# VinAIResearch/GaPro

Hardware: AMD Instinct MI355X
Metric: scenes/sec pseudo-label gen (ScanNetV2-train-shaped synthetic scenes) (higher is better)
Workload: dtype f64

## Files before the change

### gapro_amd/_lib.py

```python
from __future__ import annotations

import ctypes as C
import os
import sys
from typing import Optional

_HERE = os.path.dirname(os.path.abspath(__file__))
LIB_PATH = os.path.join(_HERE, "libgapro_hip.so")

GAPRO_OK = 0
GAPRO_ERR_BAD_ARG = -1
GAPRO_ERR_NOT_FINITE = -4
GAPRO_ERR_CHOLESKY = -5
STATUS_NAMES = {0: "OK", -1: "BAD_ARG", -2: "OOM", -3: "HIP", -4: "NOT_FINITE", -5: "CHOLESKY", -6: "SPP_RANGE",
                -7: "WORKSPACE", -8: "TIMEOUT", -9: "IO", -10: "UNSUPPORTED"}
GAPRO_ERR_WORKSPACE = -7
GAPRO_ERR_TIMEOUT = -8
GAPRO_ERR_IO = -9
GAPRO_ERR_UNSUPPORTED = -10


class GaproError(RuntimeError):
    def __init__(self, code, msg=""):
        super().__init__("libgapro_hip: %s (%d) %s" % (STATUS_NAMES.get(code, "?"), code, msg))
        self.code = code


class SceneHeader(C.Structure):
    _fields_ = [("coord_min", C.c_double * 3), ("coord_max", C.c_double * 3), ("spp_min", C.c_int64),
                ("spp_max", C.c_int64), ("feat_absmax", C.c_float), ("fixed_shift", C.c_int32),
                ("n_spps", C.c_int32), ("status", C.c_int32)]


class ScheduleCounts(C.Structure):
    _fields_ = [("n_events", C.c_int32), ("n_fits", C.c_int32), ("n_event_idx", C.c_int64),
                ("n_fit_idx", C.c_int64), ("n_fit_out", C.c_int64), ("max_m", C.c_int32), ("max_t", C.c_int32)]


class FitDesc(C.Structure):
    _fields_ = [("m1", C.c_int32), ("m2", C.c_int32), ("t", C.c_int32), ("b1", C.c_int32), ("b2", C.c_int32),
                ("scene", C.c_int32), ("slot", C.c_int32), ("reserved", C.c_int32), ("idx_offset", C.c_int64),
                ("out_offset", C.c_int64),
                ("ws_offset", C.c_int64)]


class FitLaunchStep(C.Structure):
    _fields_ = [("kernel", C.c_int32), ("variant", C.c_int32), ("first", C.c_int32), ("count", C.c_int32),
                ("grid", C.c_int32), ("stream", C.c_int32), ("ticket", C.c_int32), ("timing", C.c_int32),
                ("wait_gate", C.c_int32), ("reserved", C.c_int32), ("lds_bytes", C.c_int64)]


FIT_STEP_COPY_FREE = 8
FIT_MAX_STEPS = 10


class PredictDesc(C.Structure):
    _fields_ = [("state_offset", C.c_int64), ("row_offset", C.c_int64), ("out_offset", C.c_int64), ("t", C.c_int32),
                ("reserved", C.c_int32)]


class PointRefineScene(C.Structure):
    _fields_ = [("n_points", C.c_int64), ("n_spps", C.c_int32), ("reserved", C.c_int32), ("spp_inv", C.c_void_p),
                ("feats", C.c_void_p), ("sp_row", C.c_void_p), ("cursor", C.c_void_p), ("mu_spp", C.c_void_p),
                ("var_spp", C.c_void_p), ("sem", C.c_void_p), ("inst", C.c_void_p), ("prob", C.c_void_p),
                ("mu", C.c_void_p), ("var", C.c_void_p)]


class PointRefineModel(C.Structure):
    _fields_ = [("row_offset", C.c_int64), ("t", C.c_int32), ("scene", C.c_int32), ("sem1", C.c_int32),
                ("inst1", C.c_int32), ("sem2", C.c_int32), ("inst2", C.c_int32)]


class PointRefineBlock(C.Structure):
    _fields_ = [("row_start", C.c_int64), ("n_rows", C.c_int32), ("scene", C.c_int32), ("seg_start", C.c_int32),
                ("n_seg", C.c_int32)]


class PointRefineSegment(C.Structure):
    _fields_ = [("out_start", C.c_int64), ("model", C.c_int32), ("reserved", C.c_int32)]


class PointRefineVoteScene(C.Structure):
    _fields_ = [("sem_spp", C.c_void_p), ("inst_spp", C.c_void_p), ("prob_spp", C.c_void_p), ("mu_spp", C.c_void_p),
                ("var_spp", C.c_void_p), ("n_spps", C.c_int32), ("reserved", C.c_int32)]


class TrainsetDesc(C.Structure):
    _fields_ = [("idx_offset", C.c_int64), ("n1", C.c_int32), ("n2", C.c_int32), ("t", C.c_int32), ("m1", C.c_int32),
                ("m2", C.c_int32), ("reserved", C.c_int32), ("row_offset", C.c_int64)]


TRAINSET_POOL, TRAINSET_NEAREST = 0, 1
TRAINSET_MAX_NEAREST = 1024
TRAINSET_MAX_LIST_FACTOR = 2
TRAINSET_MAX_PROBLEMS = 32767


class SceneTask(C.Structure):
    _fields_ = [("n_points", C.c_int64), ("coords", C.c_void_p), ("feats", C.c_void_p), ("spp", C.c_void_p),
                ("spp_inv", C.c_void_p), ("prepare_ws", C.c_void_p), ("spp_range_cap", C.c_int64),
                ("boxes", C.c_void_p), ("n_boxes", C.c_int32), ("n_spps", C.c_int32), ("fixed_shift", C.c_int32),
                ("thresh_spp_occu", C.c_float), ("feat_sum", C.c_void_p), ("occ_count", C.c_void_p),
                ("point_count", C.c_void_p), ("feats_spp", C.c_void_p), ("occ_bits", C.c_void_p),
                ("n_bbs", C.c_void_p), ("sem_spp", C.c_void_p), ("inst_spp", C.c_void_p), ("prob_spp", C.c_void_p),
                ("sem", C.c_void_p), ("inst", C.c_void_p), ("prob", C.c_void_p)]


class PthArray(C.Structure):
    _fields_ = [("kind", C.c_int32), ("itemsize", C.c_int32), ("ndim", C.c_int32), ("encoded", C.c_int32),
                ("shape", C.c_int64 * 4), ("nbytes", C.c_int64)]


class InstanceHeader(C.Structure):
    _fields_ = [("instance_num", C.c_int32), ("n_boxes", C.c_int32), ("status", C.c_int32), ("reserved", C.c_int32)]


class EvalScene(C.Structure):
    _fields_ = [("point_offset", C.c_int64), ("n_points", C.c_int64), ("max_gt", C.c_int32), ("max_ps", C.c_int32),
                ("ws_offset", C.c_int64), ("row_offset", C.c_int64)]


class EvalApScene(C.Structure):
    _fields_ = [("point_offset", C.c_int64), ("n_points", C.c_int64), ("max_ps", C.c_int32), ("n_keys", C.c_int32),
                ("ws_offset", C.c_int64), ("id_offset", C.c_int64), ("key_offset", C.c_int64),
                ("pair_offset", C.c_int64)]


GAPRO_LABEL_F64, GAPRO_LABEL_I32, GAPRO_LABEL_I64 = 1, 2, 3


class InstPrepHeader(C.Structure):
    _fields_ = [("instance_num", C.c_int32), ("n_ids", C.c_int32), ("max_id", C.c_int32), ("status", C.c_int32),
                ("fixed_shift", C.c_int32), ("flags", C.c_int32)]


INST_PREP_MAX_IDS = 1 << 20
INST_PREP_GRID_CAP = 512
INST_PREP_LDS_IDS = 512


class SppGtHeader(C.Structure):
    _fields_ = [("status", C.c_int32), ("bad_sample", C.c_int32), ("flags", C.c_int32), ("batch_size", C.c_int32),
                ("total_rows", C.c_int64), ("total_cols", C.c_int64), ("total_cells", C.c_int64)]


SPP_GT_MAX_SAMPLES = 1024
SPP_GT_MAX_BATCH_SPPS = (1 << 31) - 1
SPP_GT_GRID_CAP = 512
class ProposalsInputs(C.Structure):
    _fields_ = [("n_queries", C.c_int64), ("n_voxels", C.c_int64), ("n_points", C.c_int64), ("n_spps", C.c_int32),
                ("n_mask_cols", C.c_int32), ("cls_logits", C.c_void_p), ("conf_logits", C.c_void_p),
                ("box_preds", C.c_void_p), ("mask_logits", C.c_void_p), ("voxel_spps", C.c_void_p),
                ("v2p_map", C.c_void_p), ("spps", C.c_void_p), ("semantic_preds", C.c_void_p),
                ("cand_scores", C.c_void_p), ("cand_classes", C.c_void_p), ("mask_type", C.c_int32),
                ("voxel_spps_i64", C.c_int32), ("v2p_i64", C.c_int32), ("spps_i64", C.c_int32),
                ("semantic_i64", C.c_int32), ("reserved", C.c_int32)]


PROPOSALS_MAX_PRE_TOPK, PROPOSALS_MAX_SEM2INS = 1024, 8
PROPOSALS_FULL, PROPOSALS_NMS, PROPOSALS_RLE = 0, 1, 2
PROPOSALS_NMS_MATRIX, PROPOSALS_NMS_STANDARD = 0, 1
PROPOSALS_MASK_F32, PROPOSALS_MASK_U8 = 0, 1


class ProposalsParams(C.Structure):
    _fields_ = [("mode", C.c_int32), ("instance_classes", C.c_int32), ("pre_topk", C.c_int32),
                ("type_nms", C.c_int32), ("topk", C.c_int32), ("npoint_thresh", C.c_int32),
                ("label_shift", C.c_int32), ("n_sem2ins", C.c_int32), ("logit_thresh", C.c_float),
                ("final_score_thresh", C.c_float), ("nms_threshold", C.c_float), ("reserved", C.c_int32),
                ("sem2ins_classes", C.c_int32 * PROPOSALS_MAX_SEM2INS)]


class ProposalsHeader(C.Structure):
    _fields_ = [("status", C.c_int32), ("flags", C.c_int32), ("n_rows", C.c_int32), ("n_sem2ins", C.c_int32),
                ("total_runs", C.c_int64), ("n_candidates", C.c_int32), ("n_after_npoints", C.c_int32),
                ("n_after_nms", C.c_int32), ("n_after_refine", C.c_int32)]


class SpfPredictInputs(C.Structure):
    _fields_ = [("n_queries", C.c_int64), ("n_spps", C.c_int64), ("n_points", C.c_int64), ("labels", C.c_void_p),
                ("pred_scores", C.c_void_p), ("masks", C.c_void_p), ("superpoints", C.c_void_p),
                ("coords_float", C.c_void_p), ("superpoints_i64", C.c_int32), ("reserved", C.c_int32)]


class SpfPredictParams(C.Structure):
    _fields_ = [("num_class", C.c_int32), ("topk_insts", C.c_int32), ("npoint_thr", C.c_int32),
                ("score_thr", C.c_float)]


class SpfPredictHeader(C.Structure):
    _fields_ = [("status", C.c_int32), ("flags", C.c_int32), ("n_candidates", C.c_int32), ("n_after_score", C.c_int32),
                ("n_rows", C.c_int32), ("reserved", C.c_int32), ("total_runs", C.c_int64)]


SPP_GT_HALF, SPP_GT_STRICT = 0, 1
GAPRO_ERR_SPP_RANGE = -6
GAPRO_EVAL_MAX_THRESHOLDS = 32


class MatchTask(C.Structure):
    _fields_ = [("d_mask_logits", C.c_void_p), ("ld_logits", C.c_int64), ("d_mask", C.c_void_p), ("d_cls", C.c_void_p),
                ("d_box", C.c_void_p), ("n_inst", C.c_int32), ("n_cols", C.c_int32), ("cost_offset", C.c_int64)]


class MatchWeights(C.Structure):
    _fields_ = [("w_class", C.c_double), ("w_dice", C.c_double), ("w_bce", C.c_double), ("w_conf", C.c_double),
                ("w_giou", C.c_double)]


MATCH_STATUS_WORDS = 4


class MatchLossTask(C.Structure):
    _fields_ = [("d_mask_logits", C.c_void_p), ("ld_logits", C.c_int64), ("d_inst_labels", C.c_void_p),
                ("d_cls_labels", C.c_void_p), ("d_box_labels", C.c_void_p), ("n_gt", C.c_int32), ("n_cols", C.c_int32),
                ("col_offset", C.c_int64), ("row_offset", C.c_int64)]


MATCH_LOSS_N = 7
MATCH_LOSS_MAX_FEATS = 8


class SpfLossTask(C.Structure):
    _fields_ = [("d_labels", C.c_void_p), ("d_scores", C.c_void_p), ("d_mask_logits", C.c_void_p),
                ("ld_logits", C.c_int64), ("d_gt_masks", C.c_void_p), ("d_gt_labels", C.c_void_p),
                ("d_gt_boxes", C.c_void_p), ("n_gt", C.c_int32), ("n_inst", C.c_int32), ("n_cols", C.c_int32),
                ("reserved", C.c_int32), ("col_offset", C.c_int64), ("row_offset", C.c_int64)]


class SpfLossDims(C.Structure):
    _fields_ = [("n_heads", C.c_int32), ("batch_size", C.c_int32), ("n_queries", C.c_int32), ("n_classes", C.c_int32),
                ("cls_type", C.c_int32), ("n_feats", C.c_int32), ("min_points", C.c_int32), ("flags", C.c_int32),
                ("non_object_weight", C.c_double)]


SPF_LOSS_N = 5
SPF_WEIGHTED_BCE, SPF_DICE_DIV_MAIN = 1, 2
QS_STATUS_WORDS = 4
FPS_SKIP_ORIGIN, QS_LOCAL_INDEX = 1, 2
FPS_PATHS = ("resident", "streamed", "global")
QS_MAX_SAMPLES, BALL_QUERY_MAX_NSAMPLE = 4096, 4096
VOXELIZE_MAX_ACTIVE = 4096
VOXELIZE_STATUS_WORDS = 4


SPP_SORT_TILE, SPP_MAX_SEGMENTS, SPP_MAX_BATCHES, SPP_STATUS_WORDS = 4096, 1 << 24, 65536, 4
SPP_FLAG_INDEX, SPP_FLAG_MAP, SPP_MEAN, SPP_MAX = 1, 2, 0, 1
DYCO_MAX_BATCH = 64


class SppPlan(C.Structure):
    _fields_ = [("n_points", C.c_int64), ("n_spps", C.c_int64), ("n_rows", C.c_int64), ("d_index", C.c_void_p),
                ("d_point_map", C.c_void_p), ("index_i64", C.c_int32), ("map_i64", C.c_int32),
                ("d_seg_off", C.c_void_p), ("d_seg_pts", C.c_void_p), ("d_counts", C.c_void_p),
                ("d_row_off", C.c_void_p), ("d_row_pts", C.c_void_p), ("d_seg_rows", C.c_void_p)]


class VoxelizeHeader(C.Structure):
    _fields_ = [("status", C.c_int32), ("flags", C.c_int32), ("n_voxels", C.c_int32), ("max_active", C.c_int32)]


POINT_LOSS_N = 4
POINT_LOSS_MIN_CLASSES, POINT_LOSS_MAX_CLASSES = 2, 64
POINT_LOSS_MAX_POINTS = (1 << 31) - 1
POINT_LOSS_RUN = 1024
POINT_LOSS_FOLD = 256


class FitOptions(C.Structure):
    _fields_ = [("training_iter", C.c_int32), ("lr", C.c_double), ("jitter", C.c_double),
                ("min_variance", C.c_double), ("eval_stale_chol", C.c_int32), ("reserved", C.c_int32),
                ("psd_retries", C.c_int32), ("precision", C.c_int32), ("psd_jitter", C.c_double)]


FIT_DBG_NO_STRIP = 1
FIT_DBG_CALLER_STREAM = 2
FIT_DBG_NO_SMALL = 4
FIT_DBG_NO_CLUSTER = 8
FIT_DBG_CLUSTER_ALL = 16
FIT_DBG_WG_TILED_ALL = 8192
FIT_DBG_CLUSTER_STALL = 32768
FIT_DBG_WG_TILED_NONE = 131072
FIT_DBG_STATIC_MAP = 262144
FIT_DBG_NO_WAVE = 1048576


_P = C.c_void_p
SIGNATURES = {
    "gapro_version": (C.c_int, []),
    "gapro_ctx_create": (C.c_int, [C.c_int, C.POINTER(_P)]),
    "gapro_ctx_destroy": (None, [_P]),
    "gapro_last_error": (C.c_char_p, [_P]),
    "gapro_partition_prepare_workspace_bytes": (C.c_size_t, [C.c_int64, C.c_int64]),
    "gapro_partition_prepare": (C.c_int, [_P, _P, C.c_int64, C.c_int32, _P, _P, _P, C.c_int64, _P, C.c_size_t, _P,
                                          C.POINTER(SceneHeader)]),
    "gapro_partition_prepare_async": (C.c_int, [_P, _P, C.c_int64, C.c_int32, _P, _P, _P, C.c_int64, _P, C.c_size_t,
                                                _P, _P]),
    "gapro_partition_pool": (C.c_int, [_P, _P, C.c_int64, C.c_int32, C.c_int32, C.c_int32, C.c_int32, C.c_float,
                                       _P, _P, _P, _P, _P, _P, _P, _P, _P, _P]),
    "gapro_broadcast_labels": (C.c_int, [_P, _P, C.c_int64, _P, _P, _P, _P, _P, _P, _P]),
    "gapro_partition_prepare_batch": (C.c_int, [_P, _P, C.c_int32, C.c_int32, _P, _P, _P, _P]),
    "gapro_partition_pool_batch": (C.c_int, [_P, _P, C.c_int32, C.c_int32, _P, _P]),
    "gapro_partition_pool_plan": (C.c_int, [C.c_int32, C.c_int32]),
    "gapro_broadcast_labels_batch": (C.c_int, [_P, _P, C.c_int32, _P, _P]),
    "gapro_instance_info_workspace_bytes": (C.c_size_t, [C.c_int32]),
    "gapro_instance_info": (C.c_int, [_P, _P, C.c_int64, _P, _P, _P, C.c_int32, C.c_int32, _P, C.c_size_t, _P, _P, _P, _P,
                                      _P, _P]),
    "gapro_eval_batch_workspace_bytes": (C.c_size_t, [_P, C.c_int32, C.c_int32]),
    "gapro_eval_batch": (C.c_int, [_P, _P, C.c_int32, _P, _P, C.c_int64, C.c_int32, _P, C.c_int32, _P, C.c_int32, _P,
                                   C.c_int32, _P, _P, C.c_int32, _P, C.c_int32, C.c_int32, _P, C.c_size_t, _P, _P, _P,
                                   _P, _P]),
    "gapro_eval_ap_workspace_bytes": (C.c_size_t, [_P, C.c_int32]),
    "gapro_eval_ap_keys": (C.c_int, [_P, _P, C.c_int32, _P, _P, C.c_int64, C.c_int32, _P, C.c_int32, _P, C.c_int32, _P,
                                     C.c_size_t, _P, _P]),
    "gapro_eval_ap_pair_cells": (C.c_int64, [_P, C.c_int32]),
    "gapro_eval_ap_tables": (C.c_int, [_P, _P, C.c_int32, _P, _P, C.c_int64, C.c_int32, _P, C.c_int32, _P, C.c_int32,
                                       _P, C.c_int32, _P, _P, C.c_int32, _P, C.c_size_t, _P, _P, _P, _P, _P, _P, _P,
                                       _P]),
    "gapro_eval_ap_workspace_bytes_rows": (C.c_size_t, [_P, C.c_int32, C.c_int32]),
    "gapro_eval_ap_tables_rows": (C.c_int, [_P, _P, C.c_int32, _P, _P, C.c_int64, C.c_int32, _P, C.c_int32, _P,
                                            C.c_int32, _P, C.c_int32, _P, _P, C.c_int32, _P, C.c_int32, _P, C.c_size_t,
                                            _P, _P, _P, _P, _P, _P, _P, _P]),
    "gapro_label_heuristic_workspace_bytes": (C.c_size_t, [C.c_int64, C.c_int32, C.c_int32]),
    "gapro_label_heuristic": (C.c_int, [_P, _P, C.c_int64, _P, _P, C.c_int32, C.c_int32, _P, _P, _P, C.c_int32, C.c_int32,
                                        C.c_int32, _P, C.c_size_t, _P, _P]),
    "gapro_label_pool_mean": (C.c_int, [_P, _P, C.c_int64, C.c_int32, _P, _P, _P, _P, _P, _P, _P, _P, _P]),
    "gapro_weighted_bce_with_logits": (C.c_int, [_P, _P, C.c_int32, C.c_int64, _P, _P, _P, C.c_float, _P, _P, _P]),
    "gapro_kl_gp_loss": (C.c_int, [_P, _P, C.c_int64, _P, _P, _P, _P, C.c_float, C.c_float, C.c_float, _P, _P, _P,
                                   _P]),
    "gapro_inst_prep_workspace_bytes": (C.c_size_t, [C.c_int32]),
    "gapro_inst_crop": (C.c_int, [_P, _P, C.c_int64, _P, C.c_int32, C.c_int32, _P, C.c_size_t, _P, _P]),
    "gapro_inst_info": (C.c_int, [_P, _P, C.c_int64, _P, _P, C.c_int32, _P, C.c_int32, C.c_int64, C.c_int32, _P,
                                  C.c_size_t, _P, _P, _P, _P, _P, _P, _P]),
    "gapro_inst_prepare": (C.c_int, [_P, _P, C.c_int64, _P, _P, C.c_int32, _P, C.c_int32, C.c_int64, C.c_int32, _P,
                                     C.c_size_t, _P, _P, _P, _P, _P, _P, _P]),
    "gapro_spp_gt_workspace_bytes": (C.c_size_t, [C.c_int64, C.c_int32, C.c_int32, C.c_int32]),
    "gapro_spp_gt_count": (C.c_int, [_P, _P, C.c_int64, C.c_int64, _P, C.c_int32, _P, _P, C.c_int32, C.c_int32, _P,
                                     C.c_int32, C.c_int32, _P, C.c_int32, C.c_int64, _P, C.c_size_t, _P, _P]),
    "gapro_spp_gt_fill": (C.c_int, [_P, _P, C.c_int64, C.c_int64, _P, C.c_int32, _P, _P, C.c_int32, C.c_int32, _P,
                                    C.c_int32, C.c_int32, _P, _P, C.c_int32, C.c_int64, C.c_int32, _P, C.c_size_t, _P,
                                    C.c_int64, _P, _P, _P, C.c_int64, _P]),
    "gapro_proposals_workspace_bytes": (C.c_size_t, [_P, _P]),
    "gapro_proposals_header_bytes": (C.c_size_t, [_P, _P]),
    "gapro_proposals_count": (C.c_int, [_P, _P, _P, _P, _P, C.c_size_t, _P, _P]),
    "gapro_proposals_fill": (C.c_int, [_P, _P, _P, _P, _P, C.c_size_t, _P, _P, _P, _P, C.c_int64, _P, _P, C.c_int64,
                                       _P, _P]),
    "gapro_spf_predict_workspace_bytes": (C.c_size_t, [_P, _P]),
    "gapro_spf_predict_header_bytes": (C.c_size_t, [_P, _P]),
    "gapro_spf_predict_count": (C.c_int, [_P, _P, _P, _P, _P, C.c_size_t, _P, _P]),
    "gapro_spf_predict_fill": (C.c_int, [_P, _P, _P, _P, _P, C.c_size_t, _P, _P, _P, _P, C.c_int64, _P, _P, C.c_int64,
                                         _P, _P]),
    "gapro_match_cost_workspace_bytes": (C.c_size_t, [C.c_int32, C.c_int32, C.c_int64, C.c_int64]),
    "gapro_match_cost": (C.c_int, [_P, _P, _P, C.c_int32, C.c_int32, C.c_int32, C.c_int32, _P, _P, _P, _P, _P,
                                   C.c_size_t, _P, C.c_int64, _P, _P, _P]),
    "gapro_match_loss_workspace_bytes": (C.c_size_t, [C.c_int32, C.c_int32, C.c_int64]),
    "gapro_match_loss_forward": (C.c_int, [_P, _P, _P, _P, C.c_int32, C.c_int32, C.c_int32, C.c_int32, C.c_int32, _P,
                                           _P, _P, _P, _P, _P, C.c_int64, _P, C.c_double, _P, C.c_size_t, _P, _P, _P]),
    "gapro_match_loss_backward": (C.c_int, [_P, _P, C.c_int32, C.c_int32, C.c_int32, C.c_int32, C.c_int32, C.c_int64,
                                            _P, _P, _P, _P, _P, _P, _P, C.c_double, _P, C.c_size_t, _P, _P, _P, _P,
                                            _P]),
    "gapro_spf_loss_workspace_bytes": (C.c_size_t, [C.c_int32, C.c_int32, C.c_int32, C.c_int64]),
    "gapro_spf_loss_forward": (C.c_int, [_P, _P, _P, _P, _P, _P, _P, _P, _P, C.c_int64, _P, C.c_size_t, _P, _P, _P]),
    "gapro_spf_loss_backward": (C.c_int, [_P, _P, _P, C.c_int64, _P, _P, _P, _P, C.c_size_t, _P, _P, _P, _P]),
    "gapro_point_loss_workspace_bytes": (C.c_size_t, [C.c_int64, C.c_int32]),
    "gapro_point_loss_forward": (C.c_int, [_P, _P, C.c_int64, C.c_int32, _P, C.c_int64, _P, C.c_int32, _P, C.c_int32, _P,
                                           _P, _P, _P, _P, C.c_int64, C.c_double, _P, C.c_size_t, _P, _P, _P]),
    "gapro_point_loss_backward": (C.c_int, [_P, _P, C.c_int64, C.c_int32, _P, C.c_int64, _P, C.c_int32, _P, C.c_int32, _P,
                                            _P, _P, _P, _P, C.c_int64, C.c_double, _P, C.c_size_t, _P, _P, _P, _P]),
    "gapro_fps_plan": (C.c_int, [C.c_int64, C.POINTER(C.c_int64), C.POINTER(C.c_int64)]),
    "gapro_fps_workspace_bytes": (C.c_size_t, [C.c_int64]),
    "gapro_fps_batch": (C.c_int, [_P, _P, C.c_int64, _P, C.c_int32, _P, C.c_int32, _P, C.c_int32, C.c_int64, C.c_int32,
                                  _P, C.c_size_t, _P, _P, _P, _P]),
    "gapro_ball_query_batch": (C.c_int, [_P, _P, C.c_int64, _P, C.c_int64, _P, C.c_int32, _P, C.c_int32, _P, C.c_int32,
                                         C.c_double, C.c_int32, C.c_int32, _P, _P, _P, _P]),
    "gapro_lsap_solve": (C.c_int, [C.c_int32, C.c_int32, _P, C.c_int64, C.c_int32, C.POINTER(C.c_int32), _P, _P]),
    "gapro_voxelize_table_shape": (C.c_int, [C.c_int32, C.c_int64, C.c_int64, C.POINTER(C.c_int64)]),
    "gapro_voxelize_plan": (C.c_int64, [C.c_int64]),
    "gapro_voxelize_hash": (C.c_uint64, [_P, C.c_int32]),
    "gapro_voxelize_workspace_bytes": (C.c_size_t, [C.c_int64]),
    "gapro_voxelize_count": (C.c_int, [_P, _P, C.c_int64, C.c_int32, _P, C.c_int32, _P, C.c_size_t, _P, _P, _P]),
    "gapro_voxelize_fill": (C.c_int, [_P, _P, C.c_int64, C.c_int32, _P, C.c_int32, C.c_int64, C.c_int64, _P,
                                      C.c_size_t, _P, _P, _P, _P, _P]),
    "gapro_voxelize_host_count": (C.c_int, [_P, C.c_int64, C.c_int32, C.c_int32, _P, C.POINTER(VoxelizeHeader),
                                            C.POINTER(C.c_void_p)]),
    "gapro_voxelize_host_fill": (C.c_int, [_P, _P, _P, _P, _P]),
    "gapro_voxelize_host_free": (None, [_P]),
    "gapro_voxel_pool_workspace_bytes": (C.c_size_t, [C.c_int64]),
    "gapro_voxel_pool_forward": (C.c_int, [_P, _P, C.c_int64, C.c_int32, _P, C.c_int64, C.c_int64, _P, C.c_int32,
                                           C.c_int32, _P, C.c_size_t, _P, _P, _P]),
    "gapro_voxel_pool_backward": (C.c_int, [_P, _P, C.c_int64, C.c_int32, _P, C.c_int64, C.c_int64, _P, C.c_int32, _P,
                                            _P, _P]),
    "gapro_spp_plan_workspace_bytes": (C.c_size_t, [C.c_int64, C.c_int64]),
    "gapro_spp_plan_build": (C.c_int, [_P, _P, _P, C.c_int64, _P, C.c_int32, _P, _P, C.c_size_t, _P, _P]),
    "gapro_spp_pool_forward": (C.c_int, [_P, _P, _P, _P, C.c_int64, C.c_int64, C.c_int32, C.c_int32, C.c_int32, _P, _P]),
    "gapro_spp_pool_backward": (C.c_int, [_P, _P, _P, _P, C.c_int32, C.c_int32, C.c_int32, _P, _P]),
    "gapro_dyco_param_count": (C.c_int64, [C.c_int32]),
    "gapro_dyco_workspace_bytes": (C.c_size_t, [C.c_int32, C.c_int32, C.c_int64, C.c_int32]),
    "gapro_dyco_forward": (C.c_int, [_P, _P, C.c_int32, C.c_int32, C.c_int32, _P, C.c_int64, _P, _P, C.c_int64, _P, _P,
                                     _P, _P, _P, C.c_size_t, _P]),
    "gapro_dyco_backward": (C.c_int, [_P, _P, C.c_int32, C.c_int32, C.c_int32, _P, C.c_int64, _P, _P, C.c_int64, _P, _P,
                                      _P, _P, _P, _P, C.c_size_t, _P, _P, _P, _P]),
    "gapro_schedule_build": (C.c_int, [C.c_int32, C.c_int32, _P, _P, _P, C.POINTER(_P)]),
    "gapro_schedule_free": (None, [_P]),
    "gapro_schedule_get_counts": (C.c_int, [_P, C.POINTER(ScheduleCounts)]),
    "gapro_schedule_export_fits": (C.c_int, [_P, C.c_int32, C.c_int64, C.c_int64, C.c_int32, _P, _P]),
    "gapro_schedule_export_events": (C.c_int, [_P, _P, _P, _P, _P, _P, _P]),
    "gapro_schedule_export_testers": (C.c_int, [_P, _P, _P, _P]),
    "gapro_schedule_merge": (C.c_int, [_P, _P, _P, _P, _P, _P, _P, C.c_int32, C.c_int32, _P, _P, _P, _P, _P]),
    "gapro_schedule_merge_ex": (C.c_int, [_P, _P, _P, _P, _P, _P, _P, C.c_int32, C.c_int32, _P, _P, _P, _P, _P, _P]),
    "gapro_fit_options_default": (None, [C.POINTER(FitOptions)]),
    "gapro_fit_workspace_doubles": (C.c_int64, [C.c_int32, C.c_int32, C.c_int32]),
    "gapro_fit_plan_workspace": (C.c_int64, [_P, C.c_int32, C.c_int32]),
    "gapro_svgp_fit_batch": (C.c_int, [_P, _P, C.c_int32, C.c_int32, _P, _P, _P, _P, _P, C.POINTER(FitOptions), _P,
                                       C.c_size_t, _P, _P, _P, _P, _P, _P, _P]),
    "gapro_svgp_fit_batch_ex": (C.c_int, [_P, _P, C.c_int32, C.c_int32, _P, _P, _P, _P, _P, C.POINTER(FitOptions), _P,
                                          C.c_size_t, _P, _P, _P, _P, _P, _P, _P, _P]),
    "gapro_gp_state_doubles": (C.c_int64, [C.c_int32, C.c_int32]),
    "gapro_gp_state_plan": (C.c_int64, [_P, C.c_int32, C.c_int32, _P]),
    "gapro_svgp_fit_batch_state": (C.c_int, [_P, _P, C.c_int32, C.c_int32, _P, _P, _P, _P, _P, C.POINTER(FitOptions), _P,
                                             C.c_size_t, _P, _P, _P, _P, _P, _P, _P, _P, _P, _P, C.c_size_t]),
    "gapro_svgp_predict_workspace_bytes": (C.c_size_t, [C.c_int32, C.c_int32, _P]),
    "gapro_svgp_predict_batch": (C.c_int, [_P, _P, C.c_int32, C.c_int32, _P, _P, _P, _P, C.c_int64, _P,
                                           C.POINTER(FitOptions), _P, C.c_size_t, _P, _P, _P, _P, _P, _P]),
    "gapro_point_refine_gather": (C.c_int, [_P, _P, C.c_int32, C.c_int32, _P, _P, C.c_int64, _P, _P]),
    "gapro_point_refine_apply": (C.c_int, [_P, _P, C.c_int32, _P, _P, C.c_int32, _P, _P, C.c_int64, _P, _P, _P, _P, _P,
                                           _P]),
    "gapro_point_refine_expand": (C.c_int, [_P, _P, C.c_int32, _P, _P, C.c_int32, _P, _P, C.c_int64, C.c_int64, _P]),
    "gapro_point_refine_compete": (C.c_int, [_P, _P, C.c_int32, _P, _P, C.c_int32, _P, _P, C.c_int32, _P, _P, C.c_int32,
                                             _P, _P, C.c_int64, C.c_int64, _P, _P, _P, _P, _P, _P, _P]),
    "gapro_point_refine_vote": (C.c_int, [_P, _P, C.c_int32, _P, _P, C.c_int32, _P, _P, _P, _P, C.c_int32, _P, _P, _P, _P,
                                          C.c_int32, _P, _P, C.c_int64, C.c_int64, _P, _P, _P, _P, _P, _P]),
    "gapro_spp_vote_workspace_bytes": (C.c_size_t, [C.c_int64, C.c_int32, C.c_int32]),
    "gapro_spp_vote": (C.c_int, [_P, _P, C.c_int32, C.c_int64, C.c_int32, C.c_int32, _P, _P, C.c_int32, _P, _P, _P,
                                 C.c_size_t, _P, _P, _P]),
    "gapro_trainset_workspace_bytes": (C.c_size_t, [C.c_int32, _P, C.c_int32, C.c_int32, C.c_int32]),
    "gapro_trainset_count": (C.c_int, [_P, _P, C.c_int32, C.c_int32, _P, _P, C.c_int64, C.c_int32, _P, _P, _P, C.c_size_t,
                                       _P, _P]),
    "gapro_trainset_fill": (C.c_int, [_P, _P, C.c_int32, C.c_int32, C.c_int32, _P, _P, C.c_int64, C.c_int32, _P, _P, _P,
                                      _P, C.c_int32, C.c_int32, _P, _P, C.c_size_t, C.c_int64, _P, _P, _P]),
    "gapro_fit_workspace_layout": (C.c_int, [C.c_int32, C.c_int32, C.c_int32, _P]),
    "gapro_fit_route": (C.c_int, [C.c_int32, C.c_int32]),
    "gapro_fit_route_flags": (C.c_int, [C.c_int32, C.c_int32, C.c_int32]),
    "gapro_fit_launch_plan": (C.c_int, [_P, C.c_int32, C.c_int32, C.c_int32, C.c_int32, C.POINTER(FitLaunchStep),
                                        C.c_int32, C.POINTER(C.c_int32), C.POINTER(C.c_int32)]),
    "gapro_fit_padded_m": (C.c_int, [C.c_int32, C.c_int32]),
    "gapro_fit_timing_create": (C.c_int, [_P, C.POINTER(C.c_void_p)]),
    "gapro_fit_timing_destroy": (None, [_P]),
    "gapro_fit_timing_arm": (C.c_int, [_P, _P]),
    "gapro_fit_timing_read": (C.c_int, [_P, _P, C.POINTER(C.c_float)]),
    "gapro_fit_timing_read_wave": (C.c_int, [_P, _P, C.POINTER(C.c_float)]),
    "gapro_fit_timing_offsets": (C.c_int, [_P, _P, _P, C.POINTER(C.c_float)]),
    "gapro_fit_timing_cluster_info": (C.c_int, [_P, _P, C.POINTER(C.c_int32)]),
    "gapro_pth_open": (C.c_int, [C.c_char_p, C.POINTER(_P)]),
    "gapro_pth_count": (C.c_int, [_P]),
    "gapro_pth_is_sequence": (C.c_int, [_P]),
    "gapro_pth_info": (C.c_int, [_P, C.c_int32, C.POINTER(PthArray)]),
    "gapro_pth_read": (C.c_int, [_P, C.c_int32, _P, C.c_int64]),
    "gapro_pth_close": (None, [_P]),
    "gapro_pth_write": (C.c_int, [C.c_char_p, C.c_int32, C.POINTER(PthArray), C.POINTER(_P), C.c_int32]),
    "gapro_pth_last_error": (C.c_char_p, []),
    "gapro_pth_decoder": (C.c_char_p, []),
    "gapro_pth_encoder": (C.c_char_p, []),
    "gapro_pth_crc": (C.c_char_p, []),
    "gapro_pth_crc32": (C.c_uint32, [_P, C.c_int64]),
    "gapro_pth_encode_latin1": (C.c_int64, [_P, C.c_int64, _P, C.c_int64]),
    "gapro_dev_alloc": (C.c_int, [_P, C.c_size_t, _P, C.POINTER(C.c_void_p)]),
    "gapro_dev_free": (C.c_int, [_P, _P]),
    "gapro_dev_trim": (C.c_int, [_P]),
    "gapro_dev_stats": (C.c_int, [_P, C.POINTER(C.c_int64), C.POINTER(C.c_int64), C.POINTER(C.c_int64),
                                  C.POINTER(C.c_int64)]),
    "gapro_host_alloc": (C.c_int, [_P, C.c_size_t, C.POINTER(C.c_void_p)]),
    "gapro_host_free": (C.c_int, [_P, _P]),
    "gapro_stream_create": (C.c_int, [_P, C.POINTER(C.c_void_p)]),
    "gapro_stream_destroy": (C.c_int, [_P, _P]),
    "gapro_stream_sync": (C.c_int, [_P, _P]),
    "gapro_device_sync": (C.c_int, [_P]),
    "gapro_event_create": (C.c_int, [_P, C.c_int32, C.POINTER(C.c_void_p)]),
    "gapro_event_destroy": (C.c_int, [_P, _P]),
    "gapro_event_record": (C.c_int, [_P, _P, _P]),
    "gapro_stream_wait_event": (C.c_int, [_P, _P, _P]),
    "gapro_event_sync": (C.c_int, [_P, _P]),
    "gapro_event_query": (C.c_int, [_P, _P]),
    "gapro_event_elapsed_ms": (C.c_int, [_P, _P, _P, C.POINTER(C.c_float)]),
    "gapro_memcpy_async": (C.c_int, [_P, _P, _P, C.c_size_t, C.c_int32, _P]),
    "gapro_memset_async": (C.c_int, [_P, _P, C.c_int32, C.c_size_t, _P]),
    "gapro_feed_create": (C.c_int, [C.c_int32, C.c_int32, C.c_int64, C.c_int32, C.POINTER(C.c_void_p)]),
    "gapro_feed_destroy": (None, [_P]),
    "gapro_feed_detach": (None, [_P]),
    "gapro_feed_last_error": (C.c_char_p, [_P]),
    "gapro_feed_submit": (C.c_int, [_P, C.c_int32, _P, _P, _P, _P]),
    "gapro_feed_close": (C.c_int, [_P]),
    "gapro_feed_poll": (C.c_int, [_P, C.c_int32, C.c_int32, C.c_int32, C.POINTER(C.c_int32), C.POINTER(C.c_int64)]),
    "gapro_feed_upload": (C.c_int, [_P, C.c_int32, _P, C.c_int64, _P, _P, C.POINTER(C.c_int64)]),
    "gapro_feed_batch_wait": (C.c_int, [_P, C.c_int64, _P]),
    "gapro_feed_release_batch": (C.c_int, [_P, C.c_int64]),
    "gapro_feed_export": (C.c_int, [_P, C.c_int32, _P, _P]),
    "gapro_feed_export_wait": (C.c_int, [_P, C.c_int64, C.c_int32, C.POINTER(C.c_int64), C.POINTER(C.c_int64)]),
    "gapro_feed_export_error": (C.c_int, [_P, C.c_int32, _P, C.c_int32]),
    "gapro_feed_stats": (C.c_int, [_P, _P]),
    "gapro_scene_default_feats": (C.c_int, [_P, _P, C.c_int64, _P]),
    "gapro_scene_instance_boxes": (C.c_int, [_P, _P, _P, C.c_int64, C.c_int32, C.c_int32, _P, _P, _P,
                                             C.POINTER(C.c_int32), C.POINTER(C.c_int32)]),
}

DEBUG_LIB_PATH = os.path.join(_HERE, "libgapro_hip_debug.so")
DEBUG_SIGNATURES = {
    "gapro_debug_mfma_tn": (C.c_int, [_P, _P, _P, _P, _P, C.c_int32]),
    "gapro_debug_stream": (C.c_int, [_P, _P, C.c_int64, _P, _P, C.c_int32]),
    "gapro_debug_fit_math": (C.c_int, [_P, _P, C.c_int64, _P, _P, C.c_int32]),
    "gapro_debug_mfma_peak": (C.c_int, [_P, _P, C.c_int32, C.c_int32, C.c_int32, _P, C.POINTER(C.c_double)]),
    "gapro_debug_mfma_clock": (C.c_int, [_P, _P, C.c_int32, C.c_int32, C.c_int32, _P, C.POINTER(C.c_double),
                                         C.POINTER(C.c_double)]),
    "gapro_debug_product_bench": (C.c_int, [_P, _P, C.c_int32, C.c_int32, C.c_int32, C.c_int32, C.c_int32, _P,
                                            C.POINTER(C.c_float)]),
    "gapro_debug_wgloop": (C.c_int, [_P, _P, C.c_int32, C.c_int32, C.c_int32, _P, _P, C.POINTER(C.c_double)]),
    "gapro_debug_exact_sum": (C.c_int, [_P, _P, C.c_int32, _P, _P, _P, C.c_int32, _P, _P, _P, C.c_int32, _P, _P, _P, _P]),
}

_lib: Optional[C.CDLL] = None
_dbg: Optional[C.CDLL] = None


def source_build_id() -> str:
    import glob
    import hashlib

    h = hashlib.sha256()
    files = []
    for pat in ("csrc/svgp_fit*.hip", "csrc/partition.hip", "csrc/labels.hip", "csrc/consumer.hip", "csrc/*.h"):
        files += glob.glob(os.path.join(_HERE, pat))
    for fn in sorted(files, key=os.path.basename):
        h.update(os.path.basename(fn).encode())
        with open(fn, "rb") as fh:
            h.update(fh.read())
    return h.hexdigest()[:16]


def load_debug() -> C.CDLL:
    global _dbg
    if _dbg is not None:
        return _dbg
    if not os.path.exists(DEBUG_LIB_PATH):
        raise ImportError("libgapro_hip_debug.so not built: run gapro_amd/csrc/build.sh; expected at " + DEBUG_LIB_PATH)
    lib = C.CDLL(DEBUG_LIB_PATH)
    for name, (res, args) in DEBUG_SIGNATURES.items():
        fn = getattr(lib, name)
        fn.restype = res
        fn.argtypes = args
    _dbg = lib
    return lib


_TORCH_FIRST = [True]


def load() -> C.CDLL:
    global _lib
    if _lib is not None:
        return _lib
    if not os.path.exists(LIB_PATH):
        raise ImportError("libgapro_hip.so not built: run gapro_amd/csrc/build.sh (or __graft_entry__.build()); "
                          "expected at " + LIB_PATH)
    _TORCH_FIRST[0] = "torch" in sys.modules
    lib = C.CDLL(LIB_PATH)
    default = os.path.join(_HERE, "libgapro_hip.so")
    host_only = None
    for name, (res, args) in SIGNATURES.items():
        try:
            fn = getattr(lib, name)
        except AttributeError:
            variant = os.path.abspath(LIB_PATH) != os.path.abspath(default)
            if variant and name.startswith(("gapro_gp_state_", "gapro_svgp_predict_", "gapro_svgp_fit_batch_state",
                                            "gapro_trainset_", "gapro_point_refine_", "gapro_schedule_merge_ex",
                                            "gapro_schedule_export_testers", "gapro_spp_vote",
                                            "gapro_fit_launch_plan", "gapro_inst_", "gapro_spp_gt_", "gapro_match_",
                                            "gapro_proposals_", "gapro_fps_", "gapro_ball_query_",
                                            "gapro_lsap_", "gapro_voxelize_", "gapro_voxel_pool_", "gapro_spf_predict_",
                                            "gapro_spp_plan_", "gapro_spp_pool_", "gapro_dyco_")):
                continue
            if not variant or not name.startswith(("gapro_pth_", "gapro_scene_", "gapro_feed_")):
                raise
            if host_only is None:
                host_only = C.CDLL(default)
            fn = getattr(host_only, name)
            setattr(lib, name, fn)
        fn.restype = res
        fn.argtypes = args
    _lib = lib
    return lib


class Context:

    _cache = {}

    def __init__(self, device: int = 0):
        self.lib = load()
        h = _P()
        rc = self.lib.gapro_ctx_create(int(device), C.byref(h))
        if rc != GAPRO_OK:
            raise GaproError(rc, "gapro_ctx_create(device=%d): no usable HIP device%s" % (device, (
                " (torch was imported AFTER libgapro_hip.so was loaded: the process now holds two HIP runtimes, torch's "
                "bundled one and /opt/rocm's -- import torch first, or use the torch-free backend)"
                if ("torch" in sys.modules and not _TORCH_FIRST[0]) else "")))
        self.handle = h
        self.device = int(device)
# ... 31 lines not shown
```

### gapro_amd/csrc/partition.hip

```cpp
#include <stdlib.h>

#include "common.h"
#include "exact_sum.h"
#include "launch_util.h"
#include "wave_reduce.h"

#include <algorithm>

namespace {

constexpr int kThreads = 256;
constexpr int kMaxStatBlocks = 1024;
constexpr int kScanChunk = 2048;

struct PrepareWorkspace {
  gapro_scene_header header;
  StatsPartial partials[kMaxStatBlocks];
};

static_assert(sizeof(gapro_scene_task) == 176, "gapro_scene_task layout is part of the ABI (ctypes mirror)");
constexpr size_t kFlagsOffset = (sizeof(PrepareWorkspace) + 255) / 256 * 256;

__device__ inline PrepareWorkspace* prep_ws(const gapro_scene_task& t) { return (PrepareWorkspace*)t.prepare_ws; }
__device__ inline unsigned* prep_flags(const gapro_scene_task& t) {
  return (unsigned*)((char*)t.prepare_ws + kFlagsOffset);
}
__device__ inline unsigned* prep_bsum(const gapro_scene_task& t) {
  return (unsigned*)((char*)t.prepare_ws + kFlagsOffset + ((size_t)t.spp_range_cap * sizeof(unsigned) + 255) / 256 * 256);
}

__global__ __launch_bounds__(kThreads) void k_stats(const gapro_scene_task* __restrict__ tasks, int d) {
  const gapro_scene_task& t = tasks[blockIdx.y];
  const long long n = t.n_points;
  const double* __restrict__ coords = t.coords;
  const float* __restrict__ feats = t.feats;
  const long long* __restrict__ spp = (const long long*)t.spp;
  StatsPartial* __restrict__ partials = prep_ws(t)->partials;
  const long long tid = (long long)blockIdx.x * kThreads + threadIdx.x;
  const long long stride = (long long)gridDim.x * kThreads;
  StatsPartial p = stats_identity();
  for (long long i = tid; i < n; i += stride) {
    const double x = coords[3 * i], y = coords[3 * i + 1], z = coords[3 * i + 2];
    p.mn[0] = fmin(p.mn[0], x); p.mx[0] = fmax(p.mx[0], x);
    p.mn[1] = fmin(p.mn[1], y); p.mx[1] = fmax(p.mx[1], y);
    p.mn[2] = fmin(p.mn[2], z); p.mx[2] = fmax(p.mx[2], z);
    if (!(isfinite(x) && isfinite(y) && isfinite(z))) p.fabsmax = INFINITY;
    const long long s = spp[i];
    p.smin = s < p.smin ? s : p.smin;
    p.smax = s > p.smax ? s : p.smax;
  }
  const long long nf = n * d;
  for (long long i = tid; i < nf; i += stride) {
    const float v = feats[i];
    p.fabsmax = fmaxf(p.fabsmax, isfinite(v) ? fabsf(v) : INFINITY);
  }
  p = stats_block_fold<kThreads>(p);
  if (threadIdx.x == 0) partials[blockIdx.x] = p;
}

__global__ __launch_bounds__(kThreads) void k_stats_final(const gapro_scene_task* __restrict__ tasks, int n_partials,
                                                          gapro_scene_header* __restrict__ headers) {
  const gapro_scene_task& t = tasks[blockIdx.y];
  const long long n = t.n_points, range_cap = t.spp_range_cap;
  PrepareWorkspace* ws = prep_ws(t);
  StatsPartial p = stats_identity();
  for (int j = threadIdx.x; j < n_partials; j += kThreads) stats_merge(p, ws->partials[j]);
  p = stats_block_fold<kThreads>(p);
  if (threadIdx.x != 0) return;
  gapro_scene_header h;
  for (int k = 0; k < 3; ++k) { h.coord_min[k] = p.mn[k]; h.coord_max[k] = p.mx[k]; }
  h.spp_min = p.smin; h.spp_max = p.smax; h.feat_absmax = p.fabsmax;
  h.fixed_shift = fixed_point_shift((double)p.fabsmax, n);
  h.n_spps = 0;
  h.status = GAPRO_OK;
  const unsigned long long range = (unsigned long long)p.smax - (unsigned long long)p.smin;
  if (range >= (unsigned long long)range_cap) h.status = GAPRO_ERR_SPP_RANGE;
  if (!isfinite(p.fabsmax)) h.status = GAPRO_ERR_NOT_FINITE;
  ws->header = h;
  headers[blockIdx.y] = h;
}

__global__ __launch_bounds__(kThreads) void k_clear_flags(const gapro_scene_task* __restrict__ tasks) {
  const gapro_scene_task& t = tasks[blockIdx.y];
  const PrepareWorkspace* ws = prep_ws(t);
  if (ws->header.status != GAPRO_OK) return;
  const long long range = ws->header.spp_max - ws->header.spp_min + 1;
  unsigned* __restrict__ flags = prep_flags(t);
  const long long stride = (long long)gridDim.x * kThreads;
  for (long long i = (long long)blockIdx.x * kThreads + threadIdx.x; i < range; i += stride) flags[i] = 0u;
}

__global__ __launch_bounds__(kThreads) void k_flags(const gapro_scene_task* __restrict__ tasks) {
  const gapro_scene_task& t = tasks[blockIdx.y];
  const long long n = t.n_points;
  const long long* __restrict__ spp = (const long long*)t.spp;
  const PrepareWorkspace* ws = prep_ws(t);
  unsigned* __restrict__ flags = prep_flags(t);
  if (ws->header.status != GAPRO_OK) return;
  const long long smin = ws->header.spp_min;
  const long long stride = (long long)gridDim.x * kThreads;
  for (long long i = (long long)blockIdx.x * kThreads + threadIdx.x; i < n; i += stride) flags[spp[i] - smin] = 1u;
}

__device__ inline unsigned block_exclusive_scan(unsigned v, unsigned* total) {
  __shared__ unsigned wsum[kThreads / 64];
  const int lane = threadIdx.x & 63, w = threadIdx.x >> 6;
  unsigned inc = v;
  for (int o = 1; o < 64; o <<= 1) {
    unsigned t = __shfl_up(inc, o, 64);
    if (lane >= o) inc += t;
  }
  if (lane == 63) wsum[w] = inc;
  __syncthreads();
  unsigned base = 0, tot = 0;
  for (int j = 0; j < kThreads / 64; ++j) {
    if (j < w) base += wsum[j];
    tot += wsum[j];
  }
  __syncthreads();
  *total = tot;
  return base + inc - v;
}

__global__ __launch_bounds__(kThreads) void k_scan_blocksum(const gapro_scene_task* __restrict__ tasks) {
  const gapro_scene_task& t = tasks[blockIdx.y];
  const PrepareWorkspace* ws = prep_ws(t);
  const unsigned* __restrict__ flags = prep_flags(t);
  unsigned* __restrict__ bsum = prep_bsum(t);
  if (ws->header.status != GAPRO_OK) return;
  const long long range = ws->header.spp_max - ws->header.spp_min + 1;
  const long long base = (long long)blockIdx.x * kScanChunk;
  if (base >= range) return;
  unsigned s = 0;
  for (int j = 0; j < kScanChunk / kThreads; ++j) {
    const long long i = base + (long long)threadIdx.x * (kScanChunk / kThreads) + j;
    if (i < range) s += flags[i];
  }
  unsigned tot;
  (void)block_exclusive_scan(s, &tot);
  if (threadIdx.x == 0) bsum[blockIdx.x] = tot;
}

__global__ __launch_bounds__(kThreads) void k_scan_offsets(const gapro_scene_task* __restrict__ tasks,
                                                           gapro_scene_header* __restrict__ headers) {
  const gapro_scene_task& t = tasks[blockIdx.y];
  PrepareWorkspace* ws = prep_ws(t);
  unsigned* __restrict__ bsum = prep_bsum(t);
  if (ws->header.status != GAPRO_OK) return;
  const long long range = ws->header.spp_max - ws->header.spp_min + 1;
  const int nb = (int)((range + kScanChunk - 1) / kScanChunk);
  unsigned carry = 0;
  for (int b0 = 0; b0 < nb; b0 += kThreads) {
    const int i = b0 + threadIdx.x;
    const unsigned v = i < nb ? bsum[i] : 0u;
    unsigned tot;
    const unsigned ex = block_exclusive_scan(v, &tot);
    if (i < nb) bsum[i] = carry + ex;
    carry += tot;
  }
  if (threadIdx.x == 0) {
    ws->header.n_spps = (int)carry;
    headers[blockIdx.y].n_spps = (int)carry;
  }
}

__global__ __launch_bounds__(kThreads) void k_scan_final(const gapro_scene_task* __restrict__ tasks) {
  const gapro_scene_task& t = tasks[blockIdx.y];
  const PrepareWorkspace* ws = prep_ws(t);
  unsigned* __restrict__ flags_to_rank = prep_flags(t);
  const unsigned* __restrict__ bsum = prep_bsum(t);
  if (ws->header.status != GAPRO_OK) return;
  const long long range = ws->header.spp_max - ws->header.spp_min + 1;
  const long long base = (long long)blockIdx.x * kScanChunk;
  if (base >= range) return;
  constexpr int per = kScanChunk / kThreads;
  unsigned v[per];
  unsigned s = 0;
  for (int j = 0; j < per; ++j) {
    const long long i = base + (long long)threadIdx.x * per + j;
    v[j] = i < range ? flags_to_rank[i] : 0u;
    s += v[j];
  }
  unsigned tot;
  unsigned ex = block_exclusive_scan(s, &tot) + bsum[blockIdx.x];
  for (int j = 0; j < per; ++j) {
    const long long i = base + (long long)threadIdx.x * per + j;
    if (i < range) flags_to_rank[i] = ex;
    ex += v[j];
  }
}

__global__ __launch_bounds__(kThreads) void k_rank_lookup(const gapro_scene_task* __restrict__ tasks) {
  const gapro_scene_task& t = tasks[blockIdx.y];
  const long long n = t.n_points;
  const long long* __restrict__ spp = (const long long*)t.spp;
  const PrepareWorkspace* ws = prep_ws(t);
  const unsigned* __restrict__ rank = prep_flags(t);
  int* __restrict__ spp_inv = t.spp_inv;
  if (ws->header.status != GAPRO_OK) return;
  const long long smin = ws->header.spp_min;
  const long long stride = (long long)gridDim.x * kThreads;
  for (long long i = (long long)blockIdx.x * kThreads + threadIdx.x; i < n; i += stride)
    spp_inv[i] = (int)rank[spp[i] - smin];
}

__global__ __launch_bounds__(kThreads) void k_pool_clear(const gapro_scene_task* __restrict__ tasks, int d) {
  const gapro_scene_task& t = tasks[blockIdx.y];
  const long long S = t.n_spps, nf = S * d, no = S * t.n_boxes;
  const long long stride = (long long)gridDim.x * kThreads;
  for (long long i = (long long)blockIdx.x * kThreads + threadIdx.x; i < nf + no + S; i += stride) {
    if (i < nf) t.feat_sum[i] = 0;
    else if (i < nf + no) t.occ_count[i - nf] = 0;
    else t.point_count[i - nf - no] = 0;
  }
}

__global__ __launch_bounds__(kThreads) void k_pool(const gapro_scene_task* __restrict__ tasks, int d) {
  const gapro_scene_task& t = tasks[blockIdx.y];
  const long long n = t.n_points;
  const int nb = t.n_boxes, shift = t.fixed_shift;
  const double* __restrict__ coords = t.coords;
  const float* __restrict__ feats = t.feats;
  const int* __restrict__ spp_inv = t.spp_inv;
  const double* __restrict__ boxes = t.boxes;
  unsigned long long* __restrict__ feat_sum = (unsigned long long*)t.feat_sum;
  int* __restrict__ occ_count = t.occ_count;
  int* __restrict__ point_count = t.point_count;
  extern __shared__ double sh_box[];
  for (int j = threadIdx.x; j < nb * 6; j += kThreads) {
    const int c = j % 6;
    sh_box[j] = c < 3 ? boxes[j] - 0.005 : boxes[j] + 0.005;
  }
  __syncthreads();
  const int k = threadIdx.x & (kLanesPerPoint - 1);
  const long long ppb = kThreads / kLanesPerPoint;
  const long long stride = (long long)gridDim.x * ppb;
  for (long long i = (long long)blockIdx.x * ppb + (threadIdx.x / kLanesPerPoint); i < n; i += stride) {
    const double x = coords[3 * i], y = coords[3 * i + 1], z = coords[3 * i + 2];
    const int r = spp_inv[i];
    if (k == (d & (kLanesPerPoint - 1))) atomicAdd(&point_count[r], 1);
    accumulate_features(feat_sum + (long long)r * d, feats + i * d, d, k, shift);
    int* occ_row = occ_count + (long long)r * nb;
    for (int b = k; b < nb; b += kLanesPerPoint)
      if (in_box(sh_box + 6 * b, x, y, z)) atomicAdd(&occ_row[b], 1);
  }
}

constexpr int kPoolRun = 1024;
constexpr int kProbe = 8;

__global__ __launch_bounds__(kThreads) void k_pool_lds(const gapro_scene_task* __restrict__ tasks, int d, int log2_slots,
                                                       int nb_cap) {
  const gapro_scene_task& t = tasks[blockIdx.y];
  const long long n = t.n_points;
  const long long p0 = (long long)blockIdx.x * kPoolRun;
  if (p0 >= n) return;
  const long long p1 = p0 + kPoolRun < n ? p0 + kPoolRun : n;
  const int nb = t.n_boxes, shift = t.fixed_shift;
  const double* __restrict__ coords = t.coords;
  const float* __restrict__ feats = t.feats;
  const int* __restrict__ spp_inv = t.spp_inv;
  const double* __restrict__ boxes = t.boxes;
  unsigned long long* __restrict__ feat_sum = (unsigned long long*)t.feat_sum;
  int* __restrict__ occ_count = t.occ_count;
  int* __restrict__ point_count = t.point_count;
  extern __shared__ double sh_raw[];
  const int T = 1 << log2_slots;
  double* sh_box = sh_raw;
  unsigned long long* fsum = (unsigned long long*)(sh_box + 6 * nb_cap);
  int* keys = (int*)(fsum + (size_t)T * d);
  unsigned* cnt = (unsigned*)(keys + T);
  unsigned* occ = cnt + T;
  for (int j = threadIdx.x; j < nb * 6; j += kThreads) {
    const int c = j % 6;
    sh_box[j] = c < 3 ? boxes[j] - 0.005 : boxes[j] + 0.005;
  }
  for (int j = threadIdx.x; j < T * d; j += kThreads) fsum[j] = 0ull;
  for (int j = threadIdx.x; j < T; j += kThreads) {
    keys[j] = -1;
    cnt[j] = 0u;
  }
  for (int j = threadIdx.x; j < T * nb; j += kThreads) occ[j] = 0u;
  __syncthreads();
  const int k = threadIdx.x & (kLanesPerPoint - 1);
  const int ppb = kThreads / kLanesPerPoint;
  for (long long i = p0 + (threadIdx.x / kLanesPerPoint); i < p1; i += ppb) {
    const double x = coords[3 * i], y = coords[3 * i + 1], z = coords[3 * i + 2];
    const int r = spp_inv[i];
    int slot = -1;
    unsigned h = ((unsigned)r * 2654435761u) >> (32 - log2_slots);
    for (int pr = 0; pr < kProbe; ++pr) {
      const int cur = keys[h];
      if (cur == r) { slot = (int)h; break; }
      if (cur == -1) {
        const int old = atomicCAS(&keys[h], -1, r);
        if (old == -1 || old == r) { slot = (int)h; break; }
      }
      h = (h + 1) & (unsigned)(T - 1);
    }
    const float* f = feats + i * d;
    const long long i_first = __shfl(i, 0, 64);
    const bool full_wave = i_first + 64 / kLanesPerPoint - 1 < p1;
    const bool one_spp = full_wave && __all(r == __shfl(r, 0, 64) && slot >= 0);
    if (one_spp) {
      const bool head = (threadIdx.x & 63) < kLanesPerPoint;
      if (head && k == (d & (kLanesPerPoint - 1))) atomicAdd(&cnt[slot], (unsigned)(64 / kLanesPerPoint));
      accumulate_features_wave8(fsum + (size_t)slot * d, f, d, k, shift, head);
      unsigned* occ_row = occ + (size_t)slot * nb;
      for (int b0 = 0; b0 < nb; b0 += kLanesPerPoint) {
        const int b = b0 + k;
        int in = 0;
        if (b < nb) {
          const double* bx = sh_box + 6 * b;
          in = (x >= bx[0]) & (y >= bx[1]) & (z >= bx[2]) & (x <= bx[3]) & (y <= bx[4]) & (z <= bx[5]);
        }
        in += __shfl_down(in, 8, 64);
        in += __shfl_down(in, 16, 64);
        in += __shfl_down(in, 32, 64);
        if (head && in) atomicAdd(&occ_row[b], (unsigned)in);
      }
    } else if (slot >= 0) {
      if (k == (d & (kLanesPerPoint - 1))) atomicAdd(&cnt[slot], 1u);
      accumulate_features(fsum + (size_t)slot * d, f, d, k, shift);
      unsigned* occ_row = occ + (size_t)slot * nb;
      for (int b = k; b < nb; b += kLanesPerPoint)
        if (in_box(sh_box + 6 * b, x, y, z)) atomicAdd(&occ_row[b], 1u);
    } else {
      if (k == (d & (kLanesPerPoint - 1))) atomicAdd(&point_count[r], 1);
      accumulate_features(feat_sum + (long long)r * d, f, d, k, shift);
      int* occ_row = occ_count + (long long)r * nb;
      for (int b = k; b < nb; b += kLanesPerPoint)
        if (in_box(sh_box + 6 * b, x, y, z)) atomicAdd(&occ_row[b], 1);
    }
  }
  __syncthreads();
  for (int j = threadIdx.x; j < T; j += kThreads) {
    const int r = keys[j];
    if (r >= 0 && cnt[j]) atomicAdd(&point_count[r], (int)cnt[j]);
  }
  for (int j = threadIdx.x; j < T * d; j += kThreads) {
    const int sl = j / d, c = j - sl * d;
    const int r = keys[sl];
    const unsigned long long v = fsum[j];
    if (r >= 0 && v) atomicAdd(&feat_sum[(long long)r * d + c], v);
  }
  for (int j = threadIdx.x; j < T * nb; j += kThreads) {
    const int sl = j / nb, b = j - sl * nb;
    const int r = keys[sl];
    const unsigned v = occ[j];
    if (r >= 0 && v) atomicAdd(&occ_count[(long long)r * nb + b], (int)v);
  }
}

__global__ __launch_bounds__(kThreads) void k_pool_finalize(const gapro_scene_task* __restrict__ tasks, int d) {
  const gapro_scene_task& t = tasks[blockIdx.y];
  const int n_spps = t.n_spps, nb = t.n_boxes, shift = t.fixed_shift;
  const float thresh = t.thresh_spp_occu;
  const long long* __restrict__ feat_sum = (const long long*)t.feat_sum;
  const int* __restrict__ occ_count = t.occ_count;
  const int* __restrict__ point_count = t.point_count;
  float* __restrict__ feats_spp = t.feats_spp;
  unsigned long long* __restrict__ occ_bits = (unsigned long long*)t.occ_bits;
  int* __restrict__ n_bbs = t.n_bbs;
  const int s = blockIdx.x * kThreads + threadIdx.x;
  if (s >= n_spps) return;
  const int pc = point_count[s] > 0 ? point_count[s] : 1;
  const float pcf = (float)pc;
  const int words = (nb + 63) / 64;
  int nbb = 0;
  for (int w = 0; w < words; ++w) {
    unsigned long long bits = 0;
    const int b_end = min(nb, (w + 1) * 64);
    for (int b = w * 64; b < b_end; ++b) {
      const float mean = (float)occ_count[(long long)s * nb + b] / pcf;
      if (mean >= thresh) bits |= 1ull << (b - w * 64);
    }
    occ_bits[(long long)s * words + w] = bits;
    nbb += __popcll(bits);
  }
  n_bbs[s] = nbb;
  const double pcd = (double)pc;
  for (int k = 0; k < d; ++k)
    feats_spp[(long long)s * d + k] = (float)fixed_mean(feat_sum[(long long)s * d + k], shift, pcd);
}

__global__ __launch_bounds__(kThreads) void k_broadcast(const gapro_scene_task* __restrict__ tasks) {
  const gapro_scene_task& t = tasks[blockIdx.y];
  const long long n = t.n_points;
  const int* __restrict__ spp_inv = t.spp_inv;
  const int* __restrict__ sem_spp = t.sem_spp;
  const int* __restrict__ inst_spp = t.inst_spp;
  const float* __restrict__ prob_spp = t.prob_spp;
  int* __restrict__ sem = t.sem;
  int* __restrict__ inst = t.inst;
  float* __restrict__ prob = t.prob;
  const long long stride = (long long)gridDim.x * kThreads;
  for (long long i = (long long)blockIdx.x * kThreads + threadIdx.x; i < n; i += stride) {
    const int r = spp_inv[i];
    sem[i] = sem_spp[r];
    inst[i] = inst_spp[r];
    prob[i] = prob_spp[r];
  }
}

inline size_t pool_box_bytes(int n_boxes) { return (size_t)n_boxes * 6 * sizeof(double); }
inline size_t pool_table_bytes(int feat_dim, int n_boxes, int log2_slots) {
  return ((size_t)8 + 4 * (size_t)n_boxes + 8 * (size_t)feat_dim) << log2_slots;
}

}

extern "C" {

size_t gapro_partition_prepare_workspace_bytes(int64_t n_points, int64_t spp_range_cap) {
  (void)n_points;
  if (spp_range_cap < 1) spp_range_cap = 1;
  size_t bytes = align_up(sizeof(PrepareWorkspace), 256);
  bytes += align_up((size_t)spp_range_cap * sizeof(unsigned), 256);
  bytes += align_up(((size_t)spp_range_cap / kScanChunk + 2) * sizeof(unsigned), 256);
  return bytes;
}

static int check_tasks(gapro_ctx* ctx, const char* who, int32_t n_scenes, const gapro_scene_task* h_tasks,
                       gapro_scene_task* d_tasks) {
  if (!ctx) return GAPRO_ERR_BAD_ARG;
  if (n_scenes <= 0 || n_scenes > 65535 || !h_tasks || !d_tasks)
    return gapro_fail(ctx, GAPRO_ERR_BAD_ARG, "%s: bad argument", who);
  return GAPRO_OK;
}

int gapro_partition_prepare_batch(gapro_ctx* ctx, void* stream_, int32_t n_scenes, int32_t feat_dim,
                                  const gapro_scene_task* h_tasks, gapro_scene_task* d_tasks,
                                  gapro_scene_header* d_headers, gapro_scene_header* h_headers_pinned) {
  int rc = check_tasks(ctx, "gapro_partition_prepare_batch", n_scenes, h_tasks, d_tasks);
  if (rc != GAPRO_OK) return rc;
  if (feat_dim <= 0 || !d_headers || !h_headers_pinned)
    return gapro_fail(ctx, GAPRO_ERR_BAD_ARG, "gapro_partition_prepare_batch: bad argument");
  long long n_max = 0, cap_max = 0;
  for (int i = 0; i < n_scenes; ++i) {
    const gapro_scene_task& t = h_tasks[i];
    if (t.n_points <= 0 || !t.coords || !t.feats || !t.spp || !t.spp_inv || !t.prepare_ws || t.spp_range_cap < 1)
      return gapro_fail(ctx, GAPRO_ERR_BAD_ARG, "gapro_partition_prepare_batch: scene %d: bad argument", i);
    n_max = std::max<long long>(n_max, t.n_points);
    cap_max = std::max<long long>(cap_max, t.spp_range_cap);
  }
  hipStream_t stream = (hipStream_t)stream_;
  GAPRO_HIP_CHECK(ctx, hipMemcpyAsync(d_tasks, h_tasks, (size_t)n_scenes * sizeof(gapro_scene_task),
                                      hipMemcpyHostToDevice, stream));
  const unsigned ny = (unsigned)n_scenes;
  const int g_stats = grid_for(n_max, 1, kMaxStatBlocks);
  const int g_pts = grid_for(n_max, 1, 2048);
  const int g_scan = (int)((cap_max + kScanChunk - 1) / kScanChunk);
  hipLaunchKernelGGL(k_stats, dim3(g_stats, ny), dim3(kThreads), 0, stream, d_tasks, (int)feat_dim);
  hipLaunchKernelGGL(k_stats_final, dim3(1, ny), dim3(kThreads), 0, stream, d_tasks, g_stats, d_headers);
  hipLaunchKernelGGL(k_clear_flags, dim3(grid_for(cap_max, 1, 512), ny), dim3(kThreads), 0, stream, d_tasks);
  hipLaunchKernelGGL(k_flags, dim3(g_pts, ny), dim3(kThreads), 0, stream, d_tasks);
  hipLaunchKernelGGL(k_scan_blocksum, dim3(g_scan, ny), dim3(kThreads), 0, stream, d_tasks);
  hipLaunchKernelGGL(k_scan_offsets, dim3(1, ny), dim3(kThreads), 0, stream, d_tasks, d_headers);
  hipLaunchKernelGGL(k_scan_final, dim3(g_scan, ny), dim3(kThreads), 0, stream, d_tasks);
  hipLaunchKernelGGL(k_rank_lookup, dim3(g_pts, ny), dim3(kThreads), 0, stream, d_tasks);
  GAPRO_LAUNCH_CHECK(ctx);
  GAPRO_HIP_CHECK(ctx, hipMemcpyAsync(h_headers_pinned, d_headers, (size_t)n_scenes * sizeof(gapro_scene_header),
                                      hipMemcpyDeviceToHost, stream));
  return GAPRO_OK;
}

int gapro_partition_pool_plan(int32_t feat_dim, int32_t n_boxes_max) {
  if (feat_dim <= 0 || n_boxes_max <= 0) return GAPRO_ERR_BAD_ARG;
  const size_t lds = pool_box_bytes(n_boxes_max);
  if (lds > 64 * 1024) return GAPRO_ERR_BAD_ARG;
  static const bool global_only = getenv("GAPRO_POOL_GLOBAL_ATOMICS") != nullptr;
  if (global_only) return 0;
  int log2_slots = 6;
  while (log2_slots > 4 && lds + pool_table_bytes(feat_dim, n_boxes_max, log2_slots) > 60 * 1024) --log2_slots;
  return lds + pool_table_bytes(feat_dim, n_boxes_max, log2_slots) <= 60 * 1024 ? log2_slots : 0;
}

int gapro_partition_pool_batch(gapro_ctx* ctx, void* stream_, int32_t n_scenes, int32_t feat_dim,
                               const gapro_scene_task* h_tasks, gapro_scene_task* d_tasks) {
  int rc = check_tasks(ctx, "gapro_partition_pool_batch", n_scenes, h_tasks, d_tasks);
  if (rc != GAPRO_OK) return rc;
  long long n_max = 0, clear_max = 0;
  int nb_max = 0, s_max = 0;
  for (int i = 0; i < n_scenes; ++i) {
    const gapro_scene_task& t = h_tasks[i];
    if (t.n_points <= 0 || feat_dim <= 0 || t.n_boxes <= 0 || t.n_spps <= 0 || !t.coords || !t.feats || !t.spp_inv ||
        !t.boxes || !t.feat_sum || !t.occ_count || !t.point_count || !t.feats_spp || !t.occ_bits || !t.n_bbs)
      return gapro_fail(ctx, GAPRO_ERR_BAD_ARG, "gapro_partition_pool_batch: scene %d: bad argument", i);
    n_max = std::max<long long>(n_max, t.n_points);
    nb_max = std::max(nb_max, (int)t.n_boxes);
    s_max = std::max(s_max, (int)t.n_spps);
    clear_max = std::max<long long>(clear_max, (long long)t.n_spps * (feat_dim + t.n_boxes + 1));
  }
  const int plan = gapro_partition_pool_plan(feat_dim, nb_max);
  if (plan < 0) return gapro_fail(ctx, GAPRO_ERR_BAD_ARG, "gapro_partition_pool: too many boxes (%d)", nb_max);
  const size_t lds = pool_box_bytes(nb_max);
  hipStream_t stream = (hipStream_t)stream_;
  GAPRO_HIP_CHECK(ctx, hipMemcpyAsync(d_tasks, h_tasks, (size_t)n_scenes * sizeof(gapro_scene_task),
                                      hipMemcpyHostToDevice, stream));
  const unsigned ny = (unsigned)n_scenes;
  hipLaunchKernelGGL(k_pool_clear, dim3(grid_for(clear_max, 1, 256), ny), dim3(kThreads), 0, stream, d_tasks, (int)feat_dim);
  if (plan > 0) {
    const int log2_slots = plan;
    const size_t lds2 = lds + pool_table_bytes(feat_dim, nb_max, log2_slots);
    if (lds2 > 48 * 1024)
      GAPRO_HIP_CHECK(ctx, hipFuncSetAttribute((const void*)k_pool_lds, hipFuncAttributeMaxDynamicSharedMemorySize,
                                               (int)lds2));
    const unsigned gx = (unsigned)((n_max + kPoolRun - 1) / kPoolRun);
    hipLaunchKernelGGL(k_pool_lds, dim3(gx, ny), dim3(kThreads), lds2, stream, d_tasks, (int)feat_dim, log2_slots,
                       nb_max);
  } else {
    const int cap = n_scenes >= 8 ? 512 : 4096;
    hipLaunchKernelGGL(k_pool, dim3(grid_for(n_max * kLanesPerPoint, 1, cap), ny), dim3(kThreads), lds, stream, d_tasks,
                       (int)feat_dim);
  }
  hipLaunchKernelGGL(k_pool_finalize, dim3((s_max + kThreads - 1) / kThreads, ny), dim3(kThreads), 0, stream, d_tasks,
                     (int)feat_dim);
  GAPRO_LAUNCH_CHECK(ctx);
  return GAPRO_OK;
}

int gapro_broadcast_labels_batch(gapro_ctx* ctx, void* stream_, int32_t n_scenes, const gapro_scene_task* h_tasks,
                                 gapro_scene_task* d_tasks) {
  int rc = check_tasks(ctx, "gapro_broadcast_labels_batch", n_scenes, h_tasks, d_tasks);
  if (rc != GAPRO_OK) return rc;
  long long n_max = 0;
  for (int i = 0; i < n_scenes; ++i) {
    const gapro_scene_task& t = h_tasks[i];
    if (t.n_points <= 0 || !t.spp_inv || !t.sem_spp || !t.inst_spp || !t.prob_spp || !t.sem || !t.inst || !t.prob)
      return gapro_fail(ctx, GAPRO_ERR_BAD_ARG, "gapro_broadcast_labels_batch: scene %d: bad argument", i);
    n_max = std::max<long long>(n_max, t.n_points);
  }
  hipStream_t stream = (hipStream_t)stream_;
  GAPRO_HIP_CHECK(ctx, hipMemcpyAsync(d_tasks, h_tasks, (size_t)n_scenes * sizeof(gapro_scene_task),
                                      hipMemcpyHostToDevice, stream));
  hipLaunchKernelGGL(k_broadcast, dim3(grid_for(n_max, 1, n_scenes >= 8 ? 256 : 2048), (unsigned)n_scenes), dim3(kThreads),
                     0, stream, d_tasks);
  GAPRO_LAUNCH_CHECK(ctx);
  return GAPRO_OK;
}

static gapro_scene_task* ring_slot(gapro_ctx* ctx, gapro_scene_task** h_slot) {
  const unsigned i = ctx->task_pos++ % kTaskRing;
  *h_slot = ctx->h_task_ring + i;
  return ctx->d_task_ring + i;
}

int gapro_partition_prepare_async(gapro_ctx* ctx, void* stream_, int64_t n_points, int32_t feat_dim,
                                  const double* d_coords, const float* d_feats, const int64_t* d_spp,
                                  int64_t spp_range_cap, void* d_workspace, size_t workspace_bytes,
                                  int32_t* d_spp_inv, gapro_scene_header* h_header_pinned) {
  if (!ctx) return GAPRO_ERR_BAD_ARG;
  if (n_points <= 0 || feat_dim <= 0 || !d_coords || !d_feats || !d_spp || !d_workspace || !d_spp_inv ||
      !h_header_pinned || spp_range_cap < 1)
    return gapro_fail(ctx, GAPRO_ERR_BAD_ARG, "gapro_partition_prepare: bad argument");
  if (workspace_bytes < gapro_partition_prepare_workspace_bytes(n_points, spp_range_cap))
    return gapro_fail(ctx, GAPRO_ERR_WORKSPACE, "gapro_partition_prepare: workspace too small");
  gapro_scene_task* h;
  gapro_scene_task* d = ring_slot(ctx, &h);
  *h = gapro_scene_task{};
  h->n_points = n_points; h->coords = d_coords; h->feats = d_feats; h->spp = d_spp; h->spp_inv = d_spp_inv;
  h->prepare_ws = d_workspace; h->spp_range_cap = spp_range_cap;
  return gapro_partition_prepare_batch(ctx, stream_, 1, feat_dim, h, d, &((PrepareWorkspace*)d_workspace)->header,
                                       h_header_pinned);
}

int gapro_partition_prepare(gapro_ctx* ctx, void* stream_, int64_t n_points, int32_t feat_dim,
                            const double* d_coords, const float* d_feats, const int64_t* d_spp,
                            int64_t spp_range_cap, void* d_workspace, size_t workspace_bytes,
                            int32_t* d_spp_inv, gapro_scene_header* h_header) {
  if (!ctx || !h_header) return GAPRO_ERR_BAD_ARG;
  const int rc = gapro_partition_prepare_async(ctx, stream_, n_points, feat_dim, d_coords, d_feats, d_spp,
                                               spp_range_cap, d_workspace, workspace_bytes, d_spp_inv,
                                               ctx->h_header_pinned);
  if (rc != GAPRO_OK) return rc;
  GAPRO_HIP_CHECK(ctx, hipStreamSynchronize((hipStream_t)stream_));
  *h_header = *ctx->h_header_pinned;
  if (h_header->status != GAPRO_OK)
    return gapro_fail(ctx, h_header->status,
                      "gapro_partition_prepare: superpoint id range [%lld, %lld] exceeds capacity %lld",
                      (long long)h_header->spp_min, (long long)h_header->spp_max, (long long)spp_range_cap);
  return GAPRO_OK;
}

int gapro_partition_pool(gapro_ctx* ctx, void* stream_, int64_t n_points, int32_t feat_dim, int32_t n_boxes,
                         int32_t n_spps, int32_t fixed_shift, float thresh_spp_occu, const double* d_coords,
                         const float* d_feats, const int32_t* d_spp_inv, const double* d_boxes,
                         int64_t* d_feat_sum, int32_t* d_occ_count, int32_t* d_point_count, float* d_feats_spp,
                         uint64_t* d_occ_bits, int32_t* d_n_bbs) {
  if (!ctx) return GAPRO_ERR_BAD_ARG;
  gapro_scene_task* h;
  gapro_scene_task* d = ring_slot(ctx, &h);
  *h = gapro_scene_task{};
  h->n_points = n_points; h->coords = d_coords; h->feats = d_feats; h->spp_inv = (int32_t*)d_spp_inv;
  h->boxes = d_boxes; h->n_boxes = n_boxes; h->n_spps = n_spps; h->fixed_shift = fixed_shift;
  h->thresh_spp_occu = thresh_spp_occu; h->feat_sum = d_feat_sum; h->occ_count = d_occ_count;
  h->point_count = d_point_count; h->feats_spp = d_feats_spp; h->occ_bits = d_occ_bits; h->n_bbs = d_n_bbs;
  return gapro_partition_pool_batch(ctx, stream_, 1, feat_dim, h, d);
}

int gapro_broadcast_labels(gapro_ctx* ctx, void* stream_, int64_t n_points, const int32_t* d_spp_inv,
                           const int32_t* d_sem_spp, const int32_t* d_inst_spp, const float* d_prob_spp,
                           int32_t* d_sem, int32_t* d_inst, float* d_prob) {
  if (!ctx) return GAPRO_ERR_BAD_ARG;
  gapro_scene_task* h;
  gapro_scene_task* d = ring_slot(ctx, &h);
  *h = gapro_scene_task{};
  h->n_points = n_points; h->spp_inv = (int32_t*)d_spp_inv; h->sem_spp = d_sem_spp; h->inst_spp = d_inst_spp;
  h->prob_spp = d_prob_spp; h->sem = d_sem; h->inst = d_inst; h->prob = d_prob;
  return gapro_broadcast_labels_batch(ctx, stream_, 1, h, d);
}

}
```

### gapro_amd/fit_runner.py

```python
from __future__ import annotations

import os
import sys
import threading
import time
import ctypes as C
from dataclasses import dataclass
from types import SimpleNamespace
from typing import Optional, Sequence

import numpy as np

from . import _lib
from ._lib import FitDesc, PredictDesc, SceneHeader, TrainsetDesc
from .gp_model import GPModel


REPRO_SOFT = 1.0e-5


def _ptr(t) -> C.c_void_p:
    if t is None:
        return C.c_void_p(0)
    if hasattr(t, "data_ptr"):
# ... 244 lines not shown
            oo += 4
            base += 2 * m
        it, prof = self.opt.training_iter, self.profile_fit
        self.opt.training_iter, self.profile_fit = 2, False
        try:
            self.fit_descs(feats, descs, len(sizes), np.concatenate(idx), oo, raise_on_failure=False)
        finally:
            self.opt.training_iter, self.profile_fit = it, prof

    def prealloc_workspace(self, n_bytes: int, slot: str = "shared"):
        with self.be.device_ctx():
            self._workspace(slot, max(1, int(n_bytes) // 8), headroom=1.0)

    def _workspace(self, slot: str, n_doubles: int, headroom: Optional[float] = None):
        with self._ws_lock:
            self._ws.setdefault(slot, None)
            cur = self._ws[slot]
            if cur is None or cur.numel() < n_doubles:
                if self._last_fit_done is not None:
                    self._last_fit_done.synchronize()
                size = int(n_doubles * (self.workspace_headroom if headroom is None else headroom)) + 1024
                if slot.endswith("retry"):
                    self._ws[slot] = self.be.zeros(n_doubles + 1024, self.be.f64)
                    self.be.current_stream().synchronize()
                    return self._ws[slot][:n_doubles]
                if self.trace is not None:
                    self.trace.append((time.perf_counter(), 0, "workspace grows to %.1f GB per slot" % (8e-9 * size)))
                for k in list(self._ws):
                    if k != slot and (self._ws[k] is None or k.endswith("retry")):
                        continue
                    if self._ws[k] is None or self._ws[k].numel() < size:
                        self._ws[k] = None
                        self._ws[k] = self.be.zeros(size, self.be.f64)
                self.be.current_stream().synchronize()
                if self.trace is not None:
                    self.trace.append((time.perf_counter(), 0, "workspace ready"))
            return self._ws[slot][:n_doubles]

    def _predict_launch(self, d_state, h_m: np.ndarray, descs, feats, d_rows, no: int):
        lib, ctx, be = self.lib, self.ctx, self.be
        n, D, R = len(h_m), int(feats.shape[1]), int(feats.shape[0])
        ws_bytes = int(lib.gapro_svgp_predict_workspace_bytes(n, D, _ptr(h_m)))
        ws = be.empty(ws_bytes)
        out = be.empty(block_bytes(ROW_FIELDS, no))
        o = block_views(ROW_FIELDS, out, no, be)
        stat = be.empty(n * 4)
        ctx.check(lib.gapro_svgp_predict_batch(
            ctx.handle, self._sh(), n, D, _ptr(d_state), _ptr(h_m), C.cast(descs, C.c_void_p), _ptr(feats), R,
            _ptr(d_rows), C.byref(self.opt), _ptr(ws), ws_bytes, _ptr(o["probs"]), _ptr(o["probs_new"]),
            _ptr(o["labels"]), _ptr(o["mu"]), _ptr(o["var"]), _ptr(stat)))
        return out, stat

    def predict_models(self, models: Sequence[GPModel], feats, rows: Sequence, raise_on_failure: bool = True):
        be = self.be
        n = len(models)
        D, R = int(feats.shape[1]), int(feats.shape[0])
        rows = [np.ascontiguousarray(_to_np(r, np.int64).reshape(-1)) for r in rows]
        if len(rows) != n:
            raise ValueError("predict_models: %d models but %d row vectors" % (n, len(rows)))
        pre = np.zeros(n, dtype=np.int32)
        for i, (mo, r) in enumerate(zip(models, rows)):
            if mo.d != D:
                if raise_on_failure:
                    raise ValueError("predict_models: model %d was trained at feature width %d, the features have %d"
                                     % (i, mo.d, D))
                pre[i] = -1
            elif mo.status != 0:
                if raise_on_failure:
                    raise ValueError("predict_models: model %d comes from a failed fit (status %d)" % (i, mo.status))
                pre[i] = mo.status
            if len(r) and (r.min() < 0 or r.max() >= R):
                raise ValueError("predict_models: rows of model %d reach outside the %d feature rows" % (i, R))
        live = [i for i in range(n) if pre[i] == 0]
        offsets = np.zeros(n + 1, dtype=np.int64)
        offsets[1:] = np.cumsum([len(r) for r in rows])
        tot = int(offsets[-1])
        res = dict({k: np.zeros(tot, getattr(_NP, t)) for k, t in ROW_FIELDS}, status=pre.copy(), offsets=offsets)
        if not live:
            return res
        nl = len(live)
        states = [models[i].to_state() for i in live]
        descs = (PredictDesc * nl)()
        h_m = np.array([models[i].m for i in live], dtype=np.int32)
        so = ro = 0
        for k, i in enumerate(live):
            d = descs[k]
            d.state_offset, d.row_offset, d.out_offset, d.t, d.reserved = so, ro, ro, len(rows[i]), 0
            so += len(states[k])
            ro += len(rows[i])
        no = max(ro, 1)
        d_state = be.from_numpy(np.concatenate(states))
        h_rows = np.concatenate([rows[i] for i in live]).astype(np.int32) if ro else np.zeros(1, np.int32)
        d_rows = be.from_numpy(h_rows)
        out, stat = self._predict_launch(d_state, h_m, descs, feats, d_rows, no)
        flat = block_views(ROW_FIELDS, _host(out), no)
        st = _host(stat).view(np.int32)
        ro = 0
        for k, i in enumerate(live):
            t = len(rows[i])
            res["status"][i] = st[k]
            if st[k] != _lib.GAPRO_ERR_CHOLESKY:
                for key in flat:
                    res[key][offsets[i]:offsets[i] + t] = flat[key][ro:ro + t]
            ro += t
        if raise_on_failure and (res["status"] != 0).any():
            bad = int(np.nonzero(res["status"])[0][0])
            raise _lib.GaproError(int(res["status"][bad]), "prediction of model %d of %d failed" % (bad, n))
        return res

    def _stage(self, name: str):
        ev = self.stage_events
        if ev is not None:
            e = self.be.event(enable_timing=True)
            e.record(self.be.current_stream())
            ev.append((name, e))

    def _to_device(self, x, np_dtype, be_dtype):
        if self.be.name == "torch" and hasattr(x, "is_cuda"):
            return x.to(device=self.be.device, dtype=be_dtype).contiguous()
        return self.be.from_numpy(_to_np(x, np_dtype))

    def train_sets(self, coords, feats, spp, descs, h_idx: np.ndarray, npoint_nearest: int = 800,
                   spp_pool: bool = True) -> TrainSets:
        lib, ctx, be = self.lib, self.ctx, self.be
        P = len(descs)
        d_coords = self._to_device(coords, np.float64, be.f64)
        d_feats = self._to_device(feats, np.float32, be.f32)
        d_spp = self._to_device(spp, np.int64, be.i64)
        N, D = int(d_feats.shape[0]), int(d_feats.shape[1])
        if tuple(d_coords.shape) != (N, 3) or int(d_spp.numel()) != N:
            raise ValueError("coords_float must be [N, 3], feats [N, D] and spp [N] for one N")
        self._stage("start")
        cap = max(4 * N, 1 << 20)
        pbytes = int(lib.gapro_partition_prepare_workspace_bytes(N, cap))
        prep_ws = be.empty(pbytes)
        spp_inv = be.empty(4 * N)
        hdr = SceneHeader()
        rc = lib.gapro_partition_prepare(ctx.handle, self._sh(), N, D, _ptr(d_coords), _ptr(d_feats), _ptr(d_spp), cap,
                                         _ptr(prep_ws), pbytes, _ptr(spp_inv), C.byref(hdr))
        if rc != 0 and not (rc == _lib.GAPRO_ERR_NOT_FINITE and not spp_pool):
            ctx.check(rc)
        self._stage("prepare")
        mode = _lib.TRAINSET_POOL if spp_pool else _lib.TRAINSET_NEAREST
        S = max(int(hdr.n_spps), 1)
        d_idx = be.from_numpy(h_idx)
        d_descs = be.empty(P * C.sizeof(TrainsetDesc))
        ws_bytes = int(lib.gapro_trainset_workspace_bytes(mode, C.cast(descs, C.c_void_p), P, S, D))
        ws = be.empty(ws_bytes)
        status = be.empty(4 * P)
        if spp_pool:
            counts = be.empty(8 * P)
            ctx.check(lib.gapro_trainset_count(ctx.handle, self._sh(), P, D, C.cast(descs, C.c_void_p), _ptr(d_descs), N,
                                               S, _ptr(spp_inv), _ptr(d_idx), _ptr(ws), ws_bytes, _ptr(counts),
                                               _ptr(status)))
            h_counts = _host(counts).view(np.int32)
        rows = 0
        for i in range(P):
            d = descs[i]
            d.m1 = int(h_counts[2 * i]) if spp_pool else min(int(d.n1), int(npoint_nearest))
            d.m2 = int(h_counts[2 * i + 1]) if spp_pool else min(int(d.n2), int(npoint_nearest))
            d.row_offset = rows
            rows += d.m1 + d.m2
        train = be.empty(4 * rows * D)
        sel = be.empty(8 * rows)
        ctx.check(lib.gapro_trainset_fill(ctx.handle, self._sh(), mode, P, D, C.cast(descs, C.c_void_p), _ptr(d_descs), N,
                                          S, _ptr(d_coords), _ptr(d_feats), _ptr(d_spp), _ptr(spp_inv),
                                          int(hdr.fixed_shift), int(npoint_nearest), _ptr(d_idx), _ptr(ws), ws_bytes,
                                          rows, _ptr(train), _ptr(sel), _ptr(status)))
        self._stage("assemble")
        return TrainSets(train=train.view(be.f32).view(rows, D), sel=sel.view(be.i64), status=status.view(be.i32),
                         descs=descs, n_rows=rows, d_idx=d_idx, feats=d_feats,
                         keep=(d_coords, d_spp, spp_inv, prep_ws, ws, d_descs))

    def fit_points(self, coords, feats, spp, descs, h_idx: np.ndarray, npoint_nearest: int = 800, spp_pool: bool = True,
                   keep_models: bool = False, raise_on_failure: bool = True):
        ts = self.train_sets(coords, feats, spp, descs, h_idx, npoint_nearest, spp_pool)
        P = len(descs)
        fd = (FitDesc * P)()
        pd = (PredictDesc * P)()
        fidx, io, oo = [], 0, 0
        offsets = np.zeros(P + 1, dtype=np.int64)
        for i in range(P):
            t, f = descs[i], fd[i]
            m = int(t.m1 + t.m2)
            f.m1, f.m2, f.t, f.b1, f.b2, f.scene = t.m1, t.m2, 1, 0, 1, i
            f.idx_offset, f.out_offset, f.ws_offset = io, i, 0
            fidx.append(np.arange(t.row_offset, t.row_offset + m + 1, dtype=np.int32))
            fidx[-1][m] = t.row_offset
            io += m + 1
            q = pd[i]
            q.row_offset, q.out_offset, q.t, q.reserved = t.idx_offset + t.n1 + t.n2, oo, t.t, 0
            oo += int(t.t)
            offsets[i + 1] = oo
        fidx = np.concatenate(fidx)
        h_m = np.array([descs[i].m1 + descs[i].m2 for i in range(P)], dtype=np.int32)
        no = max(oo, 1)
        flags0, prof = self.opt.reserved, self.profile_fit
        try:
            for attempt in range(2):
                pend = self.fit_launch(ts.train, fd, P, fidx, P, keep_models=True, state_to_host=keep_models)
                self._stage("fit")
                for i in range(P):
                    pd[i].state_offset = int(pend.state_off[i])
                out, pstat = self._predict_launch(pend.d_state, h_m, pd, ts.feats, ts.d_idx, no)
                self._stage("predict")
                flat = block_views(ROW_FIELDS, _host(out), no)
                st_pred = _host(pstat).view(np.int32)
                st_asm = _host(ts.status).view(np.int32)
                fit = self.fit_collect(pend, raise_on_failure=False)
                timed_out = fit["status"] == _lib.GAPRO_ERR_TIMEOUT
                if attempt or not timed_out.any() or not self.retry_timeouts:
                    break
                print("[gapro_amd] %d GP fit(s) timed out at a cluster barrier; retrying on one workgroup each"
                      % int(timed_out.sum()), file=sys.stderr)
                self.timeout_retries += int(timed_out.sum())
                self.opt.reserved = (int(flags0) | _lib.FIT_DBG_NO_CLUSTER) & ~_lib.FIT_DBG_CLUSTER_STALL
                self.profile_fit = False
        finally:
            self.opt.reserved, self.profile_fit = flags0, prof
        status = np.where(st_asm != 0, st_asm, np.where(fit["status"] != 0, fit["status"], st_pred)).astype(np.int32)
        res = {k: flat[k][:oo].copy() for k in flat}
        for i in np.nonzero(status)[0]:
            for k in flat:
                res[k][offsets[i]:offsets[i + 1]] = 0
        res.update(status=status, offsets=offsets, loss=fit["loss"], train_sets=ts)
        if keep_models:
            res["models"] = fit["models"]
        if raise_on_failure and (status != 0).any():
            bad = int(np.nonzero(status)[0][0])
            raise _lib.GaproError(int(status[bad]), "point-level fit %d of %d failed" % (bad, P))
        return res

    def fit_descs(self, feats_spp, descs, n_fits: int, h_idx: np.ndarray, n_out: int,
                  init_mean: Optional[np.ndarray] = None, keep_debug: bool = False, raise_on_failure: bool = True,
                  keep_models: bool = False):
        res = self.fit_collect(self.fit_launch(feats_spp, descs, n_fits, h_idx, n_out, init_mean, keep_debug,
                                               keep_models=keep_models), raise_on_failure=False)
        res = self._retry_timeouts(res, feats_spp, descs, h_idx, n_out, init_mean=init_mean)
        if raise_on_failure and (res["status"] != 0).any():
            bad = int(np.nonzero(res["status"])[0][0])
            raise _lib.GaproError(int(res["status"][bad]), "fit %d of %d failed" % (bad, n_fits))
        return res

    def reproducibility_probe(self, feats_spp, descs, n_fits: int, h_idx: np.ndarray, n_out: int, res=None,
                              init_mean: Optional[np.ndarray] = None, rel: float = 1e-11):
        if res is None:
            res = self.fit_descs(feats_spp, descs, n_fits, h_idx, n_out, init_mean=init_mean, raise_on_failure=False)
        jit = float(self.opt.jitter)
        self.opt.jitter = jit * (1.0 + rel)
        try:
            r2 = self.fit_descs(feats_spp, descs, n_fits, h_idx, n_out, init_mean=init_mean, raise_on_failure=False)
        finally:
            self.opt.jitter = jit
        dv, dp = np.zeros(n_fits), np.zeros(n_fits)
        for k in range(n_fits):
            d = descs[k]
            a, b = int(d.out_offset), int(d.out_offset) + int(d.t)
            if b > a:
                v1, v2 = res["var"][a:b].astype(np.float64), r2["var"][a:b].astype(np.float64)
                dv[k] = float(np.max(np.abs(v1 - v2) / np.maximum(np.abs(v1), 1e-30)))
                dp[k] = float(np.max(np.abs(res["probs"][a:b].astype(np.float64) - r2["probs"][a:b].astype(np.float64))))
        return dv, dp

    def _retry_timeouts(self, res, feats_spp, descs, h_idx, n_out, init_mean=None, slot="s0", scene_keys=None,
                        keep_state=False):
        bad = np.nonzero(res["status"] == _lib.GAPRO_ERR_TIMEOUT)[0]
        if not len(bad) or not self.retry_timeouts:
            return res
        sub = (FitDesc * len(bad))()
        for k, i in enumerate(bad):
            C.memmove(C.byref(sub, k * C.sizeof(FitDesc)), C.byref(descs, int(i) * C.sizeof(FitDesc)), C.sizeof(FitDesc))
        print("[gapro_amd] %d GP fit(s) timed out at a cluster barrier; retrying them on one workgroup each"
              % len(bad), file=sys.stderr)
        old, prof = self.opt.reserved, self.profile_fit
        self.opt.reserved = (int(old) | _lib.FIT_DBG_NO_CLUSTER) & ~_lib.FIT_DBG_CLUSTER_STALL
        self.profile_fit = False
        try:
            pend = self.fit_launch(feats_spp, sub, len(bad), h_idx, n_out, init_mean, slot=slot + "retry",
                                   scene_keys=scene_keys, keep_models=keep_state or "models" in res,
                                   state_to_host="models" in res)
            r2 = self.fit_collect(pend, raise_on_failure=False)
        finally:
            self.opt.reserved, self.profile_fit = old, prof
            with self._ws_lock:
                self._ws.pop(slot + "retry", None)
        for k, i in enumerate(bad):
            d = descs[int(i)]
            a, b = int(d.out_offset), int(d.out_offset) + int(d.t)
            for key, _ in ROW_FIELDS:
                res[key][a:b] = r2[key][a:b]
            for key, _ in FIT_FIELDS:
                res[key][i] = r2[key][k]
            if "models" in res:
                res["models"][int(i)] = r2["models"][k]
        self.timeout_retries += len(bad)
        res["retried"] = [int(i) for i in bad]
        if keep_state:
            res["retry_state"] = (pend.d_state, [int(pend.state_off[k]) for k in range(len(bad))])
        return res

    def fit_launch(self, feats_spp, descs, n_fits: int, h_idx: np.ndarray, n_out: int,
                   init_mean: Optional[np.ndarray] = None, keep_debug: bool = False, slot: str = "s0",
                   scene_keys: Optional[Sequence[int]] = None, keep_models: bool = False,
                   state_to_host: bool = True) -> PendingFit:
        lib, ctx, be = self.lib, self.ctx, self.be
        D = int(feats_spp.shape[1])
        ws_bytes = int(lib.gapro_fit_plan_workspace(C.cast(descs, C.c_void_p), n_fits, D))
        if init_mean is None and self.init_mean_std > 0.0:
            init_mean = np.zeros(len(h_idx))
            for k in range(n_fits):
                d = descs[k]
                key = int(scene_keys[d.scene]) if scene_keys is not None else int(d.scene)
                rng = np.random.default_rng([self.seed, key & 0xFFFFFFFF, int(d.b1), int(d.b2)])
                m = int(d.m1 + d.m2)
                init_mean[d.idx_offset:d.idx_offset + m] = self.init_mean_std * rng.standard_normal(m)
        d_descs = be.empty(n_fits * C.sizeof(FitDesc))
        d_idx = be.from_numpy(h_idx)
        d_init = be.from_numpy(np.ascontiguousarray(init_mean, dtype=np.float64)) if init_mean is not None else None
        ws_slot = "shared" if (self.serialize_fits and not keep_debug and not slot.endswith("retry")) else slot
        ws = self._workspace(ws_slot, ws_bytes // 8)
        no = max(n_out, 1)
        out = be.empty(block_bytes(ROW_FIELDS, no))
        stat = be.empty(block_bytes(FIT_FIELDS, n_fits))
        o, s = block_views(ROW_FIELDS, out, no, be), block_views(FIT_FIELDS, stat, n_fits, be)
        if self.profile_fit:
            tm = C.c_void_p()
            ctx.check(lib.gapro_fit_timing_create(ctx.handle, C.byref(tm)))
            ctx.check(lib.gapro_fit_timing_arm(ctx.handle, tm))
        prev = self._last_fit_done if self.serialize_fits else None
        if prev is not None:
            be.current_stream().wait_event(prev)
        args = (ctx.handle, self._sh(), n_fits, D, _ptr(feats_spp), _ptr(d_idx), C.cast(descs, C.c_void_p),
                _ptr(d_descs), _ptr(d_init), C.byref(self.opt), _ptr(ws), ws_bytes, _ptr(o["probs"]),
                _ptr(o["probs_new"]), _ptr(o["labels"]), _ptr(o["mu"]), _ptr(o["var"]), _ptr(s["status"]),
                _ptr(s["loss"]), _ptr(s["cond"]))
        d_state, state_off, state_bytes = None, None, 0
        if not keep_models:
            ctx.check(lib.gapro_svgp_fit_batch_ex(*args))
        else:
            state_off = np.zeros(max(n_fits, 1), dtype=np.int64)
            state_bytes = int(lib.gapro_gp_state_plan(C.cast(descs, C.c_void_p), n_fits, D, _ptr(state_off)))
            d_state = be.empty(max(state_bytes, 8))
            ctx.check(lib.gapro_svgp_fit_batch_state(*args, _ptr(d_state), _ptr(state_off), state_bytes))
        if self.profile_fit:
            raw = _desc_table(descs, n_fits)
            m = (raw[:, 0] + raw[:, 1]).copy()
            self.fit_events.append(FitTiming(ctx, tm, fit_flops_by_class(descs, n_fits, D, int(self.opt.training_iter),
                                                                         int(self.opt.reserved)), m))
            self.last_fit_m = m
        h_out = self._pinned(slot + "fit_out", out.numel())
        h_stat = self._pinned(slot + "fit_stat", stat.numel())
        h_out[:out.numel()].copy_(out, non_blocking=True)
        h_stat[:stat.numel()].copy_(stat, non_blocking=True)
        h_state = None
        if d_state is not None and state_to_host:
            h_state = self._pinned(slot + "fit_state", max(state_bytes, 8))
            h_state[:max(state_bytes, 8)].copy_(d_state, non_blocking=True)
        done = be.event()
        done.record(be.current_stream())
        self._last_fit_done = done
        keep = (d_descs, d_idx, d_init, ws, out, stat, feats_spp, d_state)
        return PendingFit(done=done, h_out=h_out, h_stat=h_stat, no=no, n_fits=n_fits, ws_bytes=ws_bytes, keep=keep,
                          ws=ws if keep_debug else None, descs=descs if keep_debug else None, h_state=h_state,
                          state_off=state_off, state_bytes=state_bytes, d_state=d_state)

    def fit_collect(self, p: PendingFit, raise_on_failure: bool = True):
        p.done.synchronize()
        n_fits = p.n_fits
        per_fit = {k: v[:n_fits].copy() for k, v in block_views(FIT_FIELDS, p.h_stat.numpy(), n_fits).items()}
        st = per_fit["status"]
        if raise_on_failure and (st != 0).any():
            bad = int(np.nonzero(st)[0][0])
            raise _lib.GaproError(int(st[bad]), "fit %d of %d failed" % (bad, n_fits))
        res = {k: v.copy() for k, v in block_views(ROW_FIELDS, p.h_out.numpy(), p.no).items()}
        res.update(per_fit, ws_bytes=p.ws_bytes)
        if p.h_state is not None:
            flat = p.h_state.numpy()[:p.state_bytes].view(np.float64)
            off = p.state_off
            res["models"] = [GPModel.from_state(flat[int(off[i]):]) for i in range(n_fits)]
        if p.ws is not None:
            res["workspace"] = p.ws.clone()
            res["descs"] = p.descs
        p.keep = None
        return res
```

### gapro_amd/pipeline.py

```python
from __future__ import annotations

import os
import ctypes as C
from dataclasses import dataclass, field
from typing import Callable, Optional, Sequence

import numpy as np

from . import _lib
from ._lib import FitDesc, SceneHeader, SceneTask, ScheduleCounts
from .fit_runner import FitRunner, PendingFit, _host, _ptr, _to_np
from .gp_model import SceneFit, state_doubles
from .point_level import (BLOCK_DTYPE, SEGMENT_DTYPE, plan_point_compete, plan_point_winner,
                          point_level_kw, point_mode, refine_chain, refine_plan)


class LazyViews(dict):

    def __init__(self):
        super().__init__()
        self._specs = {}

    def spec(self, name, buf, off, nbytes, dtype, shape):
        self._specs[name] = (buf, off, nbytes, dtype, shape)
        self.pop(name, None)
        return buf.data_ptr() + off

    def __missing__(self, name):
        buf, off, nbytes, dtype, shape = self._specs[name]
        v = buf[off:off + nbytes].view(dtype).view(*shape)
        self[name] = v
        return v

    def __contains__(self, name):
        return dict.__contains__(self, name) or name in self._specs


@dataclass
class SceneJob:
    coords: object
    feats: object
    spp: object
    instance_cls: np.ndarray
    instance_box: np.ndarray
    instance_box_volume: np.ndarray
    wall_box: np.ndarray
    wall_box_volume: np.ndarray
    instance_classes: int = 18
    ground_h: float = 0.1
    thresh_spp_occu: float = 0.8
    header: Optional[SceneHeader] = None
    n_spps: int = 0
    boxes: Optional[np.ndarray] = None
    boxes_cls: Optional[np.ndarray] = None
    boxes_volume: Optional[np.ndarray] = None
    feats_row_base: int = 0
    dev: dict = field(default_factory=LazyViews)
    host: dict = field(default_factory=LazyViews)
    schedule: Optional[C.c_void_p] = None
    counts: Optional[ScheduleCounts] = None
    fit_base: int = 0
    out_base: int = 0
    outputs: Optional[tuple] = None
    error: Optional[Exception] = None
    feats_spp: Optional[np.ndarray] = None
    fits: Optional[list] = None
    winner: Optional[np.ndarray] = None
    point_fit: Optional[np.ndarray] = None
    vote_box: Optional[np.ndarray] = None
    vote_count: Optional[np.ndarray] = None
    scene_key: int = 0

    @property
    def spp_inv(self):
        return self.dev["spp_inv"] if "spp_inv" in self.dev else None

    @property
    def n_points(self):
        return int(self.coords.shape[0])

    @property
    def n_boxes(self):
        return int(self.boxes.shape[0])


def make_job(coords_float, mask_feats, spp, instance_cls, instance_box, instance_box_volume, wall_box,
             wall_box_volume, instance_classes=18, ground_h=0.1, thresh_spp_occu=0.8, device=None,
             scene_key: int = 0, backend=None) -> SceneJob:
    if backend is not None and backend.name == "native":
        def dev(x, dtype):
            if backend.is_device_array(x):
                if x.dtype != np.dtype(dtype):
                    raise ValueError("device buffer of dtype %s where %s is expected" % (x.dtype, np.dtype(dtype)))
                return x
            return backend.from_numpy(np.ascontiguousarray(np.asarray(x), dtype=dtype))

        f64, f32, i64 = np.float64, np.float32, np.int64
    else:
        import torch

        device = torch.device(device if device is not None else "cuda:0")

        def dev(x, dtype):
            t = x if isinstance(x, torch.Tensor) else torch.from_numpy(np.ascontiguousarray(np.asarray(x)))
            return t.to(device=device, dtype=dtype, non_blocking=True).contiguous()

        f64, f32, i64 = torch.float64, torch.float32, torch.int64
    coords = dev(coords_float, f64)
    feats = dev(mask_feats, f32)
    if feats.dim() != 2 or coords.dim() != 2 or coords.shape[1] != 3 or feats.shape[0] != coords.shape[0]:
        raise ValueError("coords_float must be [N,3] and mask_feats [N,D]")
    sp = dev(spp, i64).reshape(-1)
    if sp.shape[0] != coords.shape[0]:
        raise ValueError("spp must have one id per point")
    ibox = _to_np(instance_box, np.float32).reshape(-1, 6)
    has_wall = wall_box is not None and len(wall_box) > 0
    return SceneJob(coords, feats, sp, _to_np(instance_cls, np.int64).reshape(-1), ibox,
                    _to_np(instance_box_volume, np.float32).reshape(-1),
                    _to_np(wall_box, np.float32).reshape(-1, 6) if has_wall else np.zeros((0, 6), np.float32),
                    _to_np(wall_box_volume, np.float32).reshape(-1) if has_wall else np.zeros((0,), np.float32),
                    int(instance_classes), float(ground_h), float(thresh_spp_occu), scene_key=int(scene_key))


@dataclass
class BatchState:
    jobs: list
    all_jobs: list
    stream: object
    slot: str
    mark: Callable
    tasks: object
    d_tasks: object
    keep_debug: bool = False
    keep_models: bool = False
    feats_spp_all: object = None
    n_fits: int = 0
    n_out: int = 0
    descs: object = None
    h_idx: Optional[np.ndarray] = None
    pending: Optional[PendingFit] = None


class Pipeline(FitRunner):
    def __init__(self, device=0, training_iter=50, init_mean_std=0.0, seed=0, eval_stale_chol=False,
                 spp_range_cap=None, force_staged=False, precision="f64", cluster_all=False, backend="torch",
                 point_level=False):
        mode = point_mode(point_level)
        super().__init__(device, training_iter, init_mean_std, seed, eval_stale_chol, force_staged, precision,
                         cluster_all, backend)
        self.spp_range_cap = spp_range_cap
        self.point_level = mode is not None
        self.point_mode = mode
        self.point_outputs = mode in ("winner", "compete")
        if self.point_level and not self.serialize_fits:
            raise ValueError("point_level needs serialised fit launches (GAPRO_OVERLAP_FITS is set)")
        self.last_refine = {}
        self._ident_rows = None
        self.strict = True
        self.last_stats = {}
        self.part_events = []
        self.profile_stages = False
        self.stage_times = {}
        self._pin_events = {}
        self._keep = {}


    def _task_array(self, jobs: Sequence[SceneJob]):
        tasks = (SceneTask * len(jobs))()
        for t, job in zip(tasks, jobs):
            t.n_points = job.n_points
            t.coords, t.feats, t.spp = job.coords.data_ptr(), job.feats.data_ptr(), job.spp.data_ptr()
        d_tasks = self.be.empty(len(jobs) * C.sizeof(SceneTask))
        return tasks, d_tasks

    @staticmethod
    def _carve(sizes, align=256):
        offs, tot = [], 0
        for sz in sizes:
            offs.append(tot)
            tot += (int(sz) + align - 1) // align * align
        return offs, max(tot, align)

    def _part_event(self, jobs, name):
        if not self.profile_fit:
            return None
        e0 = self.be.event(enable_timing=True)
        e0.record(self.be.current_stream())
        return dict(name=name, start=e0, points=sum(j.n_points for j in jobs), feat_dim=int(jobs[0].feats.shape[1]))

    def _part_event_end(self, ev):
        if ev is not None:
            ev["end"] = self.be.event(enable_timing=True)
            ev["end"].record(self.be.current_stream())
            self.part_events.append(ev)

    def _prepare_finish(self, job: SceneJob, hdr: SceneHeader):
        if hdr.status != 0:
            msg = "scene has a non-finite coordinate or feature" if hdr.status == _lib.GAPRO_ERR_NOT_FINITE else \
                "superpoint id range [%d, %d] exceeds the rank table (%d slots)" % (hdr.spp_min, hdr.spp_max,
                                                                                    job.host["range_cap"])
            job.error = _lib.GaproError(int(hdr.status), msg)
            if self.strict:
                raise job.error
            return
        job.header = hdr
        job.n_spps = int(hdr.n_spps)
        job.dev.pop("prep_ws", None)
        st = job.host.get("_static")
        if st is None:
            nw = len(job.wall_box)
            st = (np.concatenate([job.instance_box.astype(np.float64), job.wall_box.astype(np.float64),
                                  np.zeros((1, 6))], 0),
                  np.ascontiguousarray(np.concatenate([job.instance_cls,
                                                       np.full(nw + 1, job.instance_classes, dtype=np.int64)])),
                  np.concatenate([job.instance_box_volume.astype(np.float64), job.wall_box_volume.astype(np.float64),
                                  np.zeros(1)]))
            dict.__setitem__(job.host, "_static", st)
        mn, mx = hdr.coord_min, hdr.coord_max
        boxes, vol = st[0].copy(), st[2].copy()
        boxes[-1] = (mn[0], mn[1], mn[2], mx[0], mx[1], mn[2] + job.ground_h)
        floor = boxes[-1]
        vol[-1] = max(floor[3] - floor[0], 0.001) * max(floor[4] - floor[1], 0.001) * max(floor[5] - floor[2], 0.001)
        job.boxes, job.boxes_cls, job.boxes_volume = boxes, st[1], vol

    def _prepare(self, job: SceneJob):
        self._prepare_all([job])

    def _prepare_all(self, jobs: Sequence[SceneJob]):
        lib, be = self.lib, self.be
        tasks, d_tasks = self._task_array(jobs)
        D = int(jobs[0].feats.shape[1])
        caps = [int(self.spp_range_cap) if self.spp_range_cap else max(4 * j.n_points, 1 << 20) for j in jobs]
        ws_off, ws_tot = self._carve([lib.gapro_partition_prepare_workspace_bytes(j.n_points, c)
                                      for j, c in zip(jobs, caps)])
        prep_ws = be.empty(ws_tot)
        inv_off, inv_tot = self._carve([4 * j.n_points for j in jobs])
        spp_inv_all = be.empty(inv_tot)
        hsz = C.sizeof(SceneHeader)
        d_headers = be.empty(len(jobs) * hsz)
        pinned = self._pinned("headers%x" % int(be.current_stream().cuda_stream), len(jobs) * hsz)
        for t, job, cap, wo, io in zip(tasks, jobs, caps, ws_off, inv_off):
            t.spp_inv = job.dev.spec("spp_inv", spp_inv_all, io, 4 * job.n_points, be.i32, (job.n_points,))
            dict.__setitem__(job.host, "range_cap", cap)
            t.prepare_ws, t.spp_range_cap = prep_ws.data_ptr() + wo, cap
        ev = self._part_event(jobs, "prepare")
        self.ctx.check(lib.gapro_partition_prepare_batch(
            self.ctx.handle, self._sh(), len(jobs), D, C.cast(tasks, C.c_void_p), _ptr(d_tasks),
            _ptr(d_headers), _ptr(pinned)))
        self._part_event_end(ev)
        be.current_stream().synchronize()
        raw = pinned.numpy()
        for i, job in enumerate(jobs):
            self._prepare_finish(job, SceneHeader.from_buffer_copy(raw[i * hsz:(i + 1) * hsz].tobytes()))
        good = [i for i, job in enumerate(jobs) if job.error is None]
        if len(good) != len(jobs):
            tasks2 = (SceneTask * max(len(good), 1))()
            for k, i in enumerate(good):
                tasks2[k] = tasks[i]
            tasks = tasks2
            d_tasks = be.empty(max(len(good), 1) * C.sizeof(SceneTask))
        return tasks, d_tasks

    def _pool(self, job: SceneJob, feats_spp_all, stage=None, off: int = 0):
        tasks, d_tasks = self._task_array([job])
        tasks[0].spp_inv = job.spp_inv.data_ptr()
        self._pool_all([job], tasks, d_tasks, feats_spp_all, stage)

    def _pool_all(self, jobs: Sequence[SceneJob], tasks, d_tasks, feats_spp_all, stage=None):
        lib, be = self.lib, self.be
        D = int(jobs[0].feats.shape[1])
        box_off, box_tot = self._carve([j.boxes.nbytes for j in jobs], 64)
        slot = "%x" % int(be.current_stream().cuda_stream)
        h_boxes = self._pinned("boxes" + slot, box_tot)
        hb = h_boxes.numpy()
        for job, bo in zip(jobs, box_off):
            hb[bo:bo + job.boxes.nbytes] = job.boxes.view(np.uint8).reshape(-1)
        d_boxes = be.empty(box_tot)
        d_boxes.copy_(h_boxes[:box_tot], non_blocking=True)
        pl = 4 if self.point_level else 0
        tab_sizes = [j.n_spps * (((j.n_boxes + 63) // 64) * 8 + 4 + pl) for j in jobs]
        tab_off, tab_tot = self._carve(tab_sizes, 16)
        d_tables = be.empty(tab_tot)
        tal_sizes = [j.n_spps * (8 * D + 4 * j.n_boxes + 4 - pl) for j in jobs]
        tal_off, tal_tot = self._carve(tal_sizes, 16)
        d_tallies = be.empty(tal_tot)
        if stage is None:
            stage = be.pinned(tab_tot)
        fbase, fstride = feats_spp_all.data_ptr(), 4 * D
        for t, job, bo, to, ao in zip(tasks, jobs, box_off, tab_off, tal_off):
            S, B = job.n_spps, job.n_boxes
            W = (B + 63) // 64
            d = job.dev
            t.boxes = d.spec("boxes", d_boxes, bo, job.boxes.nbytes, be.f64, (B, 6))
            t.feat_sum = d.spec("feat_sum", d_tallies, ao, 8 * S * D, be.i64, (S, D))
            t.occ_count = d.spec("occ_count", d_tallies, ao + 8 * S * D, 4 * S * B, be.i32, (S, B))
            if pl:
                t.point_count = d.spec("point_count", d_tables, to + 8 * S * W + 4 * S, 4 * S, be.i32, (S,))
            else:
                t.point_count = d.spec("point_count", d_tallies, ao + 8 * S * D + 4 * S * B, 4 * S, be.i32, (S,))
            t.occ_bits = d.spec("occ_bits", d_tables, to, 8 * S * W, be.i64, (S, W))
            t.n_bbs = d.spec("n_bbs", d_tables, to + 8 * S * W, 4 * S, be.i32, (S,))
            t.feats_spp = fbase + job.feats_row_base * fstride
            dict.__setitem__(d, "feats_spp", None)
            d._specs["feats_spp"] = (feats_spp_all.view(be.u8).view(-1), job.feats_row_base * fstride, S * fstride,
                                     be.f32, (S, D))
            dict.pop(d, "feats_spp", None)
            t.n_boxes, t.n_spps = B, S
            t.fixed_shift, t.thresh_spp_occu = int(job.header.fixed_shift), float(job.thresh_spp_occu)
            h = job.host
            h.spec("occ_bits_pin", stage, to, 8 * S * W, be.i64, (S, W))
            h.spec("n_bbs_pin", stage, to + 8 * S * W, 4 * S, be.i32, (S,))
            if pl:
                h.spec("point_count_pin", stage, to + 8 * S * W + 4 * S, 4 * S, be.i32, (S,))
        ev = self._part_event(jobs, "pool")
        self.ctx.check(lib.gapro_partition_pool_batch(self.ctx.handle, self._sh(), len(jobs), D,
                                                      C.cast(tasks, C.c_void_p), _ptr(d_tasks)))
        self._part_event_end(ev)
        stage[:tab_tot].copy_(d_tables, non_blocking=True)

    def _host_threads(self):
        if getattr(self, "_host_pool", None) is None:
            import concurrent.futures as cf

            self._host_pool = cf.ThreadPoolExecutor(max_workers=max(2, min(16, (os.cpu_count() or 4) // 8)))
        return self._host_pool

    def _schedule(self, job: SceneJob):
        h = job.host
        h["occ_bits"] = np.ascontiguousarray(h["occ_bits_pin"].numpy().view(np.uint64))
        h["n_bbs"] = np.ascontiguousarray(h["n_bbs_pin"].numpy())
        if "point_count_pin" in h:
            h["point_count"] = h["point_count_pin"].numpy().copy()
        sched = C.c_void_p()
        rc = self.lib.gapro_schedule_build(job.n_spps, job.n_boxes, _ptr(job.boxes), _ptr(h["occ_bits"]),
                                           _ptr(h["n_bbs"]), C.byref(sched))
        if rc != 0:
            raise _lib.GaproError(rc, "gapro_schedule_build")
        job.schedule = sched
        cnt = ScheduleCounts()
        self.lib.gapro_schedule_get_counts(sched, C.byref(cnt))
        job.counts = cnt

    def run(self, jobs: Sequence[SceneJob], keep_debug: bool = False, keep_models: bool = False):
        return self._finish(self._start(jobs, keep_debug, keep_models))

    kSlots = 3

    def _ensure_streams(self):
        if not hasattr(self, "_streams"):
            self._streams = [self.be.new_stream() for _ in range(self.kSlots)]
            for st in self._streams:
                self._ws.setdefault("s%x" % int(st.cuda_stream), None)

    def run_pipelined(self, batches: Sequence[Sequence[SceneJob]]):
        self._ensure_streams()
        ready = self.be.current_stream().record_event()
        for st in self._streams:
            st.wait_event(ready)
        outs = list(self._stream_batches(iter(batches)))
        for st in self._streams:
            self.be.current_stream().wait_stream(st)
        return outs

    def run_stream(self, batches):
        self._ensure_streams()
        ready = self.be.current_stream().record_event()
        for st in self._streams:
            st.wait_event(ready)
        for i, out in enumerate(self._stream_batches(iter(batches))):
            self.be.current_stream().wait_stream(self._streams[i % self.kSlots])
            yield out

    def _stream_batches(self, it):
        S = self.kSlots

        def on(k, fn, *a):
            with self.be.stream(self._streams[k % S]):
                return fn(*a)

        cur = on(0, next, it, None)
        if cur is None:
            return
        i = 0
        cur_state = on(0, self._partition, cur, False)
        on(0, self._schedule_all, cur_state)
        on(0, self._launch, cur_state)
        nxt = on(1, next, it, None)
        prev_state = None
        while cur_state is not None:
            nxt_state = on(i + 1, self._partition, nxt, False) if nxt is not None else None
            early = None
            if self.point_level and prev_state is not None:
                early = on(i - 1, self._finish, prev_state, False)
            if i > 0:
                on(i, self._launch, cur_state)
            if prev_state is not None:
                yield early if early is not None else on(i - 1, self._finish, prev_state, False)
            nxt = on(i + 2, next, it, None) if nxt is not None else None
            if nxt_state is not None:
                on(i + 1, self._schedule_all, nxt_state)
            prev_state, cur_state = cur_state, nxt_state
            i += 1
        yield on(i - 1, self._finish, prev_state, True)

    def _start(self, jobs: Sequence[SceneJob], keep_debug: bool = False, keep_models: bool = False):
        state = self._partition(jobs, keep_debug)
        state.keep_models = keep_models
        self._schedule_all(state)
        self._launch(state)
        return state

    def _marker(self, jobs):
        import time as _time
        t = [_time.perf_counter()]

        def _mark(name):
            if self.trace is not None:
                self.trace.append((_time.perf_counter(), id(jobs) & 0xFFFF, name))
            if self.profile_stages:
                self.be.synchronize()
                now = _time.perf_counter()
                self.stage_times[name] = self.stage_times.get(name, 0.0) + (now - t[0])
                t[0] = now

        return _mark

    def _partition(self, jobs: Sequence[SceneJob], keep_debug: bool = False):
        _mark = self._marker(jobs)
        stream = self.be.current_stream()
        slot = "s%x" % int(stream.cuda_stream)
        _mark("start")
        all_jobs = list(jobs)
        tasks, d_tasks = self._prepare_all(jobs)
        jobs = [j for j in all_jobs if j.error is None]
        _mark("A prepare")
        if not jobs:
            return BatchState([], all_jobs, stream, slot, _mark, tasks, d_tasks, keep_debug)
        D = int(jobs[0].feats.shape[1])
        base = 0
        for job in jobs:
            if int(job.feats.shape[1]) != D:
                raise ValueError("all scenes of a batch must share the feature dimension")
            job.feats_row_base = base
            base += job.n_spps
        feats_spp_all = self.be.empty_typed((base, D), self.be.f32)
        need = sum(job.n_spps * (((job.n_boxes + 63) // 64) * 8 + 4 + (4 if self.point_level else 0)) + 16
                   for job in jobs)
        stage = self._pinned(slot + "tables", need)
        self._pool_all(jobs, tasks, d_tasks, feats_spp_all, stage)
        stream.synchronize()
        _mark("B pool")
        return BatchState(jobs, all_jobs, stream, slot, _mark, tasks, d_tasks, keep_debug, feats_spp_all=feats_spp_all)

    def _schedule_all(self, state: BatchState):
        lib = self.lib
        jobs, _mark = state.jobs, state.mark
        if not jobs:
            return
        if len(jobs) >= 8:
            list(self._host_threads().map(self._schedule, jobs))
        else:
            for job in jobs:
                self._schedule(job)
        _mark("C schedule")
        n_fits = sum(j.counts.n_fits for j in jobs)
        n_idx = sum(j.counts.n_fit_idx for j in jobs)
        n_out = sum(j.counts.n_fit_out for j in jobs)
        descs = (FitDesc * max(n_fits, 1))()
        h_idx = np.zeros(max(n_idx, 1), dtype=np.int32)
        fo = io = oo = 0
        for si, job in enumerate(jobs):
            job.fit_base, job.out_base = fo, oo
            if job.counts.n_fits:
                rc = lib.gapro_schedule_export_fits(
                    job.schedule, job.feats_row_base, io, oo, si,
                    C.cast(C.byref(descs, fo * C.sizeof(FitDesc)), C.c_void_p), _ptr(h_idx[io:]))
                if rc != 0:
                    raise _lib.GaproError(rc, "gapro_schedule_export_fits")
            fo += job.counts.n_fits
            io += job.counts.n_fit_idx
            oo += job.counts.n_fit_out
        _mark("C export")
        state.n_fits, state.n_out, state.descs, state.h_idx = n_fits, n_out, descs, h_idx

    def _launch(self, state: BatchState):
        if state.n_fits:
            state.pending = self.fit_launch(state.feats_spp_all, state.descs, state.n_fits, state.h_idx, state.n_out,
                                            keep_debug=state.keep_debug, slot=state.slot,
                                            scene_keys=[j.scene_key for j in state.jobs],
                                            keep_models=state.keep_models or self.point_level,
                                            state_to_host=state.keep_models)
        state.mark("D launched")

    def _finish(self, state: BatchState, sync: bool = True):
        lib, ctx, be = self.lib, self.ctx, self.be
        jobs, keep_debug, _mark = state.jobs, state.keep_debug, state.mark
        _mark("finish")
        if not jobs:
            self.last_stats = dict(n_fits=0, n_fit_out=0, fit=None)
            return [None for _ in state.all_jobs]
        res = self.fit_collect(state.pending, raise_on_failure=False) if state.pending is not None else None
        if res is not None:
            res = self._retry_timeouts(res, state.feats_spp_all, state.descs, state.h_idx, state.n_out,
                                       slot=state.slot, scene_keys=[j.scene_key for j in jobs],
                                       keep_state=self.point_level)
            if "retry_state" in res:
                d2, off2 = res["retry_state"]
                D = int(state.feats_spp_all.shape[1])
                for k, i in enumerate(res["retried"]):
                    nb = 8 * state_doubles(int(state.descs[i].m1 + state.descs[i].m2), D)
                    a, b = 8 * int(state.pending.state_off[i]), 8 * off2[k]
                    state.pending.d_state[a:a + nb].copy_(d2[b:b + nb], non_blocking=True)
        _mark("D fit")
        if state.keep_models:
            feats_all = _host(state.feats_spp_all)
            descs, h_idx = state.descs, state.h_idx
            for job in jobs:
                job.feats_spp = feats_all[job.feats_row_base:job.feats_row_base + job.n_spps].copy()
                job.fits = []
                for k in range(job.fit_base, job.fit_base + job.counts.n_fits):
                    d = descs[k]
                    io, m = int(d.idx_offset), int(d.m1 + d.m2)
                    job.fits.append(SceneFit(int(d.b1), int(d.b2), h_idx[io:io + m] - job.feats_row_base,
                                             h_idx[io + m:io + m + int(d.t)] - job.feats_row_base, res["models"][k],
                                             int(d.m1)))
        if res is not None and (res["status"] != 0).any():
            for job in jobs:
                st = res["status"][job.fit_base:job.fit_base + job.counts.n_fits]
                if (st != 0).any():
                    k = int(np.nonzero(st)[0][0])
                    job.error = _lib.GaproError(int(st[k]), "GP fit %d of %d of the scene failed (%d failed in all)"
                                                % (k, job.counts.n_fits, int((st != 0).sum())))
            if self.strict:
                raise next(j.error for j in jobs if j.error is not None)
        want_winner = self.point_level or state.keep_models
        tot_s = sum(job.n_spps for job in jobs)
        tables = self._pinned(state.slot + "labels", tot_s * 20)
        busy = self._pin_events.pop(state.slot + "labels", None)
        if busy is not None:
            busy.synchronize()
        d_tables = be.empty(tot_s * 20)
        tab_np = tables.numpy()
        offs, off = [], 0
        for job in jobs:
            offs.append(off)
            off += 20 * job.n_spps

        def merge_one(arg):
            job, off = arg
            S = job.n_spps
            sem_spp = tab_np[off:off + 4 * S].view(np.int32)
            inst_spp = tab_np[off + 4 * S:off + 8 * S].view(np.int32)
            prob_spp = tab_np[off + 8 * S:off + 12 * S].view(np.float32)
            mu_spp = tab_np[off + 12 * S:off + 16 * S].view(np.float32)
            var_spp = tab_np[off + 16 * S:off + 20 * S].view(np.float32)
            if job.counts.n_fits:
                a, b = job.out_base, job.out_base + job.counts.n_fit_out
                pn, lb, mu, var = (res["probs_new"][a:b], res["labels"][a:b], res["mu"][a:b], res["var"][a:b])
            else:
                pn = lb = mu = var = None
            winner = np.empty(S, dtype=np.int32) if want_winner else None
            rc = lib.gapro_schedule_merge_ex(job.schedule, _ptr(pn), _ptr(lb), _ptr(mu), _ptr(var),
                                             _ptr(job.boxes_cls), _ptr(job.boxes_volume), len(job.instance_box),
                                             job.instance_classes, _ptr(sem_spp), _ptr(inst_spp), _ptr(prob_spp),
                                             _ptr(mu_spp), _ptr(var_spp), _ptr(winner))
            if rc != 0:
                raise _lib.GaproError(rc, "gapro_schedule_merge_ex")
            job.host.update(sem_spp=sem_spp.copy(), inst_spp=inst_spp.copy(), prob_spp=prob_spp.copy())
            if want_winner:
                dict.__setitem__(job.host, "winner", winner)
                if state.keep_models:
                    job.winner = winner

        if len(jobs) >= 8:
            list(self._host_threads().map(merge_one, zip(jobs, offs)))
        else:
            for arg in zip(jobs, offs):
                merge_one(arg)
        plan = refine_plan(self, state) if self.point_level else None
        d_tables.copy_(tables[:tot_s * 20], non_blocking=True)
        self._pin_events[state.slot + "labels"] = be.current_stream().record_event()
        tasks, d_tasks = state.tasks, state.d_tasks
        per_point = 20 if self.point_outputs else 12
        out_off, out_tot = self._carve([per_point * job.n_points for job in jobs], 16)
        d_out = be.empty(out_tot)
        for t, job, off, oo in zip(tasks, jobs, offs, out_off):
            S, n = job.n_spps, job.n_points
            sem = d_out[oo:oo + 4 * n].view(be.i32)
            ins = d_out[oo + 4 * n:oo + 8 * n].view(be.i32)
            prb = d_out[oo + 8 * n:oo + 12 * n].view(be.f32)
            t.sem_spp = d_tables.data_ptr() + off
            t.inst_spp = d_tables.data_ptr() + off + 4 * S
            t.prob_spp = d_tables.data_ptr() + off + 8 * S
            t.sem, t.inst, t.prob = sem.data_ptr(), ins.data_ptr(), prb.data_ptr()
            mu_spp = d_tables[off + 12 * S:off + 16 * S].view(be.f32)
            var_spp = d_tables[off + 16 * S:off + 20 * S].view(be.f32)
            if self.point_outputs:
                job.outputs = (sem, ins, prb, d_out[oo + 12 * n:oo + 16 * n].view(be.f32),
                               d_out[oo + 16 * n:oo + 20 * n].view(be.f32))
                dict.__setitem__(job.dev, "mu_var_spp", (mu_spp, var_spp))
            else:
                job.outputs = (sem, ins, prb, mu_spp, var_spp)
            if not keep_debug:
                lib.gapro_schedule_free(job.schedule)
                job.schedule = None
        refined = None
        if self.point_level and not self.point_outputs:
            refined = refine_chain(self, state, plan, offs, d_tables)
        ev = self._part_event(jobs, "broadcast")
        ctx.check(lib.gapro_broadcast_labels_batch(ctx.handle, self._sh(), len(jobs),
                                                   C.cast(tasks, C.c_void_p), _ptr(d_tasks)))
        self._part_event_end(ev)
        if refined is not None:
            self._stage("labels")
        if self.point_outputs:
            refined = refine_chain(self, state, plan, offs, d_tables)
        self._keep[state.slot] = (tasks, d_tasks, refined)
        if sync:
            be.current_stream().synchronize()
        _mark("E+F merge/broadcast")
        self.last_stats = dict(n_fits=state.n_fits, n_fit_out=state.n_out, fit=res)
        for j in jobs:
            if j.error is not None:
                j.outputs = None
        return [j.outputs if j.error is None else None for j in state.all_jobs]
```

### include/gapro_hip.h

```cpp
#ifndef GAPRO_HIP_H
#define GAPRO_HIP_H

#include <stddef.h>
#include <stdint.h>

#ifdef __cplusplus
extern "C" {
#endif

#define GAPRO_VERSION 200

typedef enum {
  GAPRO_OK = 0,
  GAPRO_ERR_BAD_ARG = -1,
  GAPRO_ERR_OOM = -2,
  GAPRO_ERR_HIP = -3,
  GAPRO_ERR_NOT_FINITE = -4,
  GAPRO_ERR_CHOLESKY = -5,
  GAPRO_ERR_SPP_RANGE = -6,
  GAPRO_ERR_WORKSPACE = -7,
  GAPRO_ERR_TIMEOUT = -8,
  GAPRO_ERR_IO = -9,
  GAPRO_ERR_UNSUPPORTED = -10
} gapro_status;

typedef struct gapro_ctx gapro_ctx;
typedef struct gapro_schedule gapro_schedule;

int gapro_version(void);
int gapro_ctx_create(int device, gapro_ctx** out);
void gapro_ctx_destroy(gapro_ctx* ctx);
const char* gapro_last_error(const gapro_ctx* ctx);


typedef struct {
  double coord_min[3];
  double coord_max[3];
  int64_t spp_min;
  int64_t spp_max;
  float feat_absmax;
  int32_t fixed_shift;
  int32_t n_spps;
  int32_t status;
} gapro_scene_header;

size_t gapro_partition_prepare_workspace_bytes(int64_t n_points, int64_t spp_range_cap);

int gapro_partition_prepare(gapro_ctx* ctx, void* stream, int64_t n_points, int32_t feat_dim,
                            const double* d_coords, const float* d_feats, const int64_t* d_spp,
                            int64_t spp_range_cap, void* d_workspace, size_t workspace_bytes,
                            int32_t* d_spp_inv, gapro_scene_header* h_header);

int gapro_partition_prepare_async(gapro_ctx* ctx, void* stream, int64_t n_points, int32_t feat_dim,
                                  const double* d_coords, const float* d_feats, const int64_t* d_spp,
                                  int64_t spp_range_cap, void* d_workspace, size_t workspace_bytes,
                                  int32_t* d_spp_inv, gapro_scene_header* h_header_pinned);

int gapro_partition_pool(gapro_ctx* ctx, void* stream, int64_t n_points, int32_t feat_dim,
                         int32_t n_boxes, int32_t n_spps, int32_t fixed_shift, float thresh_spp_occu,
                         const double* d_coords, const float* d_feats, const int32_t* d_spp_inv,
                         const double* d_boxes, int64_t* d_feat_sum, int32_t* d_occ_count,
                         int32_t* d_point_count, float* d_feats_spp, uint64_t* d_occ_bits,
                         int32_t* d_n_bbs);

int gapro_broadcast_labels(gapro_ctx* ctx, void* stream, int64_t n_points, const int32_t* d_spp_inv,
                           const int32_t* d_sem_spp, const int32_t* d_inst_spp, const float* d_prob_spp,
                           int32_t* d_sem, int32_t* d_inst, float* d_prob);

typedef struct {
  int64_t n_points;
  const double* coords;
  const float* feats;
  const int64_t* spp;
  int32_t* spp_inv;
  void* prepare_ws;
  int64_t spp_range_cap;
  const double* boxes;
  int32_t n_boxes, n_spps, fixed_shift;
  float thresh_spp_occu;
  int64_t* feat_sum;
  int32_t* occ_count;
  int32_t* point_count;
  float* feats_spp;
  uint64_t* occ_bits;
  int32_t* n_bbs;
  const int32_t* sem_spp;
  const int32_t* inst_spp;
  const float* prob_spp;
  int32_t* sem;
  int32_t* inst;
  float* prob;
} gapro_scene_task;

int gapro_partition_prepare_batch(gapro_ctx* ctx, void* stream, int32_t n_scenes, int32_t feat_dim,
                                  const gapro_scene_task* h_tasks, gapro_scene_task* d_tasks,
                                  gapro_scene_header* d_headers, gapro_scene_header* h_headers_pinned);
int gapro_partition_pool_batch(gapro_ctx* ctx, void* stream, int32_t n_scenes, int32_t feat_dim,
                               const gapro_scene_task* h_tasks, gapro_scene_task* d_tasks);
int gapro_partition_pool_plan(int32_t feat_dim, int32_t n_boxes_max);
int gapro_broadcast_labels_batch(gapro_ctx* ctx, void* stream, int32_t n_scenes,
                                 const gapro_scene_task* h_tasks, gapro_scene_task* d_tasks);

typedef struct {
  int32_t instance_num;
  int32_t n_boxes;
  int32_t status;
  int32_t reserved;
} gapro_instance_header;

size_t gapro_instance_info_workspace_bytes(int32_t max_instances);
int gapro_instance_info(gapro_ctx* ctx, void* stream, int64_t n_points, const double* d_coords,
                        const double* d_instance_label, const double* d_semantic_label, int32_t max_instances,
                        int32_t scannet_class_shift, void* d_workspace, size_t workspace_bytes, double* d_box,
                        double* d_cls, double* d_volume, float* d_corners, gapro_instance_header* d_header,
                        gapro_instance_header* h_header_pinned);

enum {
  GAPRO_LABEL_F64 = 1,
  GAPRO_LABEL_I32 = 2,
  GAPRO_LABEL_I64 = 3
};
#define GAPRO_EVAL_MAX_THRESHOLDS 32

typedef struct {
  int64_t point_offset;
  int64_t n_points;
  int32_t max_gt;
  int32_t max_ps;
  int64_t ws_offset;
  int64_t row_offset;
} gapro_eval_scene;

size_t gapro_eval_batch_workspace_bytes(gapro_eval_scene* h_scenes, int32_t n_scenes, int32_t n_thresholds);
int gapro_eval_batch(gapro_ctx* ctx, void* stream, int32_t n_scenes, const gapro_eval_scene* h_scenes,
                     gapro_eval_scene* d_scenes, int64_t n_total_points, int32_t sem_gt_dtype, const void* d_sem_gt,
                     int32_t inst_gt_dtype, const void* d_inst_gt, int32_t sem_ps_dtype, const void* d_sem_ps,
                     int32_t inst_ps_dtype, const void* d_inst_ps, const float* d_prob, int32_t n_thresholds,
                     const float* h_thresholds, int32_t scannet_remap, int32_t num_classes, void* d_workspace,
                     size_t workspace_bytes, float* d_max_iou, float* d_gt_cls, int64_t* d_conf, int64_t* d_kept,
                     int32_t* d_status);

typedef struct {
  int64_t point_offset;
  int64_t n_points;
  int32_t max_ps;
  int32_t n_keys;
  int64_t ws_offset;
  int64_t id_offset;
  int64_t key_offset;
  int64_t pair_offset;
} gapro_eval_ap_scene;

size_t gapro_eval_ap_workspace_bytes(gapro_eval_ap_scene* h_scenes, int32_t n_scenes);
int gapro_eval_ap_keys(gapro_ctx* ctx, void* stream, int32_t n_scenes, const gapro_eval_ap_scene* h_scenes,
                       gapro_eval_ap_scene* d_scenes, int64_t n_total_points, int32_t sem_gt_dtype, const void* d_sem_gt,
                       int32_t inst_gt_dtype, const void* d_inst_gt, int32_t scannet_remap, void* d_workspace,
                       size_t workspace_bytes, int32_t* d_n_keys, int32_t* d_status);
int64_t gapro_eval_ap_pair_cells(gapro_eval_ap_scene* h_scenes, int32_t n_scenes);
int gapro_eval_ap_tables(gapro_ctx* ctx, void* stream, int32_t n_scenes, const gapro_eval_ap_scene* h_scenes,
                         gapro_eval_ap_scene* d_scenes, int64_t n_total_points, int32_t sem_gt_dtype,
                         const void* d_sem_gt, int32_t inst_gt_dtype, const void* d_inst_gt, int32_t sem_ps_dtype,
                         const void* d_sem_ps, int32_t inst_ps_dtype, const void* d_inst_ps, const float* d_prob,
                         int32_t scannet_remap, void* d_workspace, size_t workspace_bytes, int32_t* d_key_code,
                         int32_t* d_key_n, int32_t* d_ps_n, int32_t* d_ps_label, int32_t* d_ps_void,
                         int64_t* d_ps_sum, int32_t* d_pair, int32_t* d_status);
size_t gapro_eval_ap_workspace_bytes_rows(gapro_eval_ap_scene* h_scenes, int32_t n_scenes, int32_t n_thresholds);
int gapro_eval_ap_tables_rows(gapro_ctx* ctx, void* stream, int32_t n_scenes, const gapro_eval_ap_scene* h_scenes,
                              gapro_eval_ap_scene* d_scenes, int64_t n_total_points, int32_t sem_gt_dtype,
                              const void* d_sem_gt, int32_t inst_gt_dtype, const void* d_inst_gt, int32_t sem_ps_dtype,
                              const void* d_sem_ps, int32_t inst_ps_dtype, const void* d_inst_ps, const float* d_prob,
                              int32_t n_thresholds, const float* h_thresholds, int32_t scannet_remap, void* d_workspace,
                              size_t workspace_bytes, int32_t* d_key_code, int32_t* d_key_n, int32_t* d_ps_n,
                              int32_t* d_ps_label, int32_t* d_ps_void, int64_t* d_ps_sum, int32_t* d_pair,
                              int32_t* d_status);

size_t gapro_label_heuristic_workspace_bytes(int64_t n_points, int32_t n_spps, int32_t n_boxes);
int gapro_label_heuristic(gapro_ctx* ctx, void* stream, int64_t n_points, const double* d_coords,
                          const int32_t* d_spp_inv, int32_t n_spps, int32_t n_boxes, const float* d_box,
                          const float* d_volume, const int64_t* d_cls, int32_t rule, int32_t align,
                          int32_t instance_classes, void* d_workspace, size_t workspace_bytes, int32_t* d_sem,
                          int32_t* d_inst);

int gapro_label_pool_mean(gapro_ctx* ctx, void* stream, int64_t n_points, int32_t n_out, const int64_t* d_index,
                          const float* d_prob, const float* d_mu, const float* d_var, double* d_sums_ws,
                          int32_t* d_counts_ws, float* d_out_prob, float* d_out_mu, float* d_out_var);
int gapro_weighted_bce_with_logits(gapro_ctx* ctx, void* stream, int32_t n_rows, int64_t n_cols, const float* d_logits,
                                   const float* d_targets, const float* d_weights, float grad_out, double* d_acc2,
                                   float* d_loss, float* d_grad_logits);
int gapro_kl_gp_loss(gapro_ctx* ctx, void* stream, int64_t n, const float* d_mu_labels, const float* d_var_labels,
                     const float* d_mu_pred, const float* d_logvar_pred, float epsilon, float weight, float grad_out,
                     double* d_acc4, float* d_loss, float* d_grad_mu, float* d_grad_logvar);

typedef struct {
  int32_t n_events;
  int32_t n_fits;
  int64_t n_event_idx;
  int64_t n_fit_idx;
  int64_t n_fit_out;
  int32_t max_m;
  int32_t max_t;
} gapro_schedule_counts;

typedef struct {
  int32_t m1, m2, t;
  int32_t b1, b2;
  int32_t scene;
  int32_t slot;
  int32_t reserved;
  int64_t idx_offset;
  int64_t out_offset;
  int64_t ws_offset;
} gapro_fit_desc;

int gapro_schedule_build(int32_t n_spps, int32_t n_boxes, const double* h_boxes,
                         const uint64_t* h_occ_bits, const int32_t* h_n_bbs, gapro_schedule** out);
void gapro_schedule_free(gapro_schedule* s);
int gapro_schedule_get_counts(const gapro_schedule* s, gapro_schedule_counts* out);
int gapro_schedule_export_fits(const gapro_schedule* s, int32_t feats_row_base, int64_t idx_base,
                               int64_t out_base, int32_t scene, gapro_fit_desc* h_descs, int32_t* h_idx);
int gapro_schedule_export_events(const gapro_schedule* s, uint8_t* h_kind, int32_t* h_b1, int32_t* h_b2,
                                 int32_t* h_aux, int64_t* h_offsets, int32_t* h_event_idx);
int gapro_schedule_export_testers(const gapro_schedule* s, int64_t* h_offsets, int32_t* h_fit, int32_t* h_pos);

int gapro_schedule_merge(const gapro_schedule* s, const float* h_probs_new, const uint8_t* h_labels,
                         const float* h_mu, const float* h_var, const int64_t* h_boxes_cls,
                         const double* h_boxes_volume, int32_t n_fg_instances, int32_t instance_classes,
                         int32_t* h_sem_spp, int32_t* h_inst_spp, float* h_prob_spp, float* h_mu_spp,
                         float* h_var_spp);
int gapro_schedule_merge_ex(const gapro_schedule* s, const float* h_probs_new, const uint8_t* h_labels,
                            const float* h_mu, const float* h_var, const int64_t* h_boxes_cls,
                            const double* h_boxes_volume, int32_t n_fg_instances, int32_t instance_classes,
                            int32_t* h_sem_spp, int32_t* h_inst_spp, float* h_prob_spp, float* h_mu_spp,
                            float* h_var_spp, int32_t* h_winner_fit);

typedef struct {
  int32_t training_iter;
  double lr;
  double jitter;
  double min_variance;
  int32_t eval_stale_chol;
  int32_t reserved;
  int32_t psd_retries;
  int32_t precision;
  double psd_jitter;
} gapro_fit_options;

enum {
  GAPRO_FIT_DBG_NO_STRIP = 1,
  GAPRO_FIT_DBG_CALLER_STREAM = 2,
  GAPRO_FIT_DBG_NO_SMALL = 4,
  GAPRO_FIT_DBG_NO_CLUSTER = 8,
  GAPRO_FIT_DBG_CLUSTER_ALL = 16,
  GAPRO_FIT_DBG_WG_TILED_ALL = 8192,
  GAPRO_FIT_DBG_CLUSTER_STALL = 32768,
  GAPRO_FIT_DBG_WG_TILED_NONE = 131072,
  GAPRO_FIT_DBG_STATIC_MAP = 262144,
  GAPRO_FIT_DBG_NO_WAVE = 1048576,
  GAPRO_FIT_DBG_ALL = 1 | 2 | 4 | 8 | 16 | 8192 | 32768 | 131072 | 262144 | 1048576
};

enum {
  GAPRO_PRECISION_F64 = 0,
  GAPRO_PRECISION_MIXED = 1
};

void gapro_fit_options_default(gapro_fit_options* opt);

int64_t gapro_fit_workspace_doubles(int32_t m, int32_t t, int32_t feat_dim);
int64_t gapro_fit_plan_workspace(gapro_fit_desc* h_descs, int32_t n_fits, int32_t feat_dim);

int gapro_svgp_fit_batch(gapro_ctx* ctx, void* stream, int32_t n_fits, int32_t feat_dim,
                         const float* d_feats_spp, const int32_t* d_idx, const gapro_fit_desc* h_descs,
                         gapro_fit_desc* d_descs, const double* d_init_mean, const gapro_fit_options* opt,
                         double* d_workspace,
                         size_t workspace_bytes, float* d_probs, float* d_probs_new, uint8_t* d_labels,
                         float* d_mu, float* d_var, int32_t* d_fit_status, double* d_fit_loss);
int gapro_svgp_fit_batch_ex(gapro_ctx* ctx, void* stream, int32_t n_fits, int32_t feat_dim,
                            const float* d_feats_spp, const int32_t* d_idx, const gapro_fit_desc* h_descs,
                            gapro_fit_desc* d_descs, const double* d_init_mean, const gapro_fit_options* opt,
                            double* d_workspace,
                            size_t workspace_bytes, float* d_probs, float* d_probs_new, uint8_t* d_labels,
                            float* d_mu, float* d_var, int32_t* d_fit_status, double* d_fit_loss, double* d_fit_cond);

int64_t gapro_gp_state_doubles(int32_t m, int32_t feat_dim);
int64_t gapro_gp_state_plan(const gapro_fit_desc* h_descs, int32_t n_fits, int32_t feat_dim, int64_t* h_state_offsets);
int gapro_svgp_fit_batch_state(gapro_ctx* ctx, void* stream, int32_t n_fits, int32_t feat_dim,
                               const float* d_feats_spp, const int32_t* d_idx, const gapro_fit_desc* h_descs,
                               gapro_fit_desc* d_descs, const double* d_init_mean, const gapro_fit_options* opt,
                               double* d_workspace, size_t workspace_bytes, float* d_probs, float* d_probs_new,
                               uint8_t* d_labels, float* d_mu, float* d_var, int32_t* d_fit_status, double* d_fit_loss,
                               double* d_fit_cond, double* d_state, const int64_t* h_state_offsets, size_t state_bytes);

typedef struct {
  int64_t state_offset;
  int64_t row_offset;
  int64_t out_offset;
  int32_t t;
  int32_t reserved;
} gapro_predict_desc;

size_t gapro_svgp_predict_workspace_bytes(int32_t n_models, int32_t feat_dim, const int32_t* h_m);
int gapro_svgp_predict_batch(gapro_ctx* ctx, void* stream, int32_t n_models, int32_t feat_dim, const double* d_state,
                             const int32_t* h_m, const gapro_predict_desc* h_descs, const float* d_feats,
                             int64_t n_feat_rows, const int32_t* d_rows, const gapro_fit_options* opt,
                             void* d_workspace, size_t workspace_bytes, float* d_probs, float* d_probs_new,
                             uint8_t* d_labels, float* d_mu, float* d_var, int32_t* d_status);

typedef struct {
  int64_t n_points;
  int32_t n_spps;
  int32_t reserved;
  const int32_t* spp_inv;
  const float* feats;
  const int64_t* sp_row;
  int32_t* cursor;
  const float* mu_spp;
  const float* var_spp;
  int32_t* sem;
  int32_t* inst;
  float* prob;
  float* mu;
  float* var;
} gapro_point_refine_scene;

typedef struct {
  int64_t row_offset;
  int32_t t;
  int32_t scene;
  int32_t sem1, inst1;
  int32_t sem2, inst2;
} gapro_point_refine_model;

int gapro_point_refine_gather(gapro_ctx* ctx, void* stream, int32_t n_scenes, int32_t feat_dim,
                              const gapro_point_refine_scene* h_scenes, gapro_point_refine_scene* d_scenes,
                              int64_t n_rows, float* d_row_feats, int32_t* d_row_point);
int gapro_point_refine_apply(gapro_ctx* ctx, void* stream, int32_t n_scenes, const gapro_point_refine_scene* h_scenes,
                             gapro_point_refine_scene* d_scenes, int32_t n_models,
                             const gapro_point_refine_model* h_models, gapro_point_refine_model* d_models,
                             int64_t n_rows, const int32_t* d_row_point, const float* d_probs_new,
                             const uint8_t* d_labels, const float* d_mu, const float* d_var,
                             const int32_t* d_model_status);

typedef struct {
  int64_t row_start;
  int32_t n_rows;
  int32_t scene;
  int32_t seg_start;
  int32_t n_seg;
} gapro_point_refine_block;

typedef struct {
  int64_t out_start;
  int32_t model;
  int32_t reserved;
} gapro_point_refine_segment;

int gapro_point_refine_expand(gapro_ctx* ctx, void* stream, int32_t n_blocks, const gapro_point_refine_block* h_blocks,
                              gapro_point_refine_block* d_blocks, int32_t n_segs,
                              const gapro_point_refine_segment* h_segs, gapro_point_refine_segment* d_segs,
                              int64_t n_rows, int64_t n_rows2, int32_t* d_rows);
int gapro_point_refine_compete(gapro_ctx* ctx, void* stream, int32_t n_scenes, const gapro_point_refine_scene* h_scenes,
                               gapro_point_refine_scene* d_scenes, int32_t n_models,
                               const gapro_point_refine_model* h_models, gapro_point_refine_model* d_models,
                               int32_t n_blocks, const gapro_point_refine_block* h_blocks,
                               gapro_point_refine_block* d_blocks, int32_t n_segs,
                               const gapro_point_refine_segment* h_segs, gapro_point_refine_segment* d_segs,
                               int64_t n_rows, int64_t n_rows2, const int32_t* d_row_point, const float* d_probs_new,
                               const uint8_t* d_labels, const float* d_mu, const float* d_var,
                               const int32_t* d_model_status, int32_t* d_row_model);

typedef struct {
  int32_t* sem_spp;
  int32_t* inst_spp;
  float* prob_spp;
  float* mu_spp;
  float* var_spp;
  int32_t n_spps;
  int32_t reserved;
} gapro_point_refine_vote_scene;

int gapro_point_refine_vote(gapro_ctx* ctx, void* stream, int32_t n_scenes,
                            const gapro_point_refine_vote_scene* h_scenes, gapro_point_refine_vote_scene* d_scenes,
                            int32_t n_models, const gapro_point_refine_model* h_models,
                            gapro_point_refine_model* d_models, const int32_t* h_model_boxes, int32_t* d_model_boxes,
                            int32_t n_blocks, const gapro_point_refine_block* h_blocks,
                            gapro_point_refine_block* d_blocks, const int32_t* h_block_spp, int32_t* d_block_spp,
                            int32_t n_segs, const gapro_point_refine_segment* h_segs,
                            gapro_point_refine_segment* d_segs, int64_t n_rows, int64_t n_rows2,
                            const float* d_probs_new, const uint8_t* d_labels, const float* d_mu, const float* d_var,
                            const int32_t* d_model_status, int32_t* d_block_out);

enum { GAPRO_VOTE_ALIGN = 0, GAPRO_VOTE_MAJOR = 1 };
size_t gapro_spp_vote_workspace_bytes(int64_t n_points, int32_t n_spps, int32_t n_classes);
int gapro_spp_vote(gapro_ctx* ctx, void* stream, int32_t mode, int64_t n_points, int32_t n_spps, int32_t n_classes,
                   const int32_t* d_ids, const void* d_label, int32_t label_is_i64, const float* d_prob,
                   const uint8_t* d_gate, void* d_ws, size_t ws_bytes, int64_t* d_label_out, float* d_prob_out,
                   int32_t* d_status);

#define GAPRO_INST_PREP_MAX_IDS 1048576
#define GAPRO_INST_PREP_GRID_CAP 512
#define GAPRO_INST_PREP_LDS_IDS 512
// ... 546 lines not shown
```

Measured before the change: 380.3.

## Fuse partition prepare and pool on device with on-GPU arena layout

Adds a device-side layout kernel that scans the per-scene superpoint counts from the prepare headers. It carves the pool tallies, tables and feature buffers out of preallocated arenas and patches the task pointers and ground box rows on the GPU. Prepare and pool can then be enqueued back to back without a host round-trip to read headers and allocate buffers. The finalize kernel becomes grid-stride because superpoint counts are not known on the host at launch, so grids are sized from point counts. The risks are arena overflow, which falls back to the old path, and more launched but idle blocks.

```diff
diff --git a/gapro_amd/_lib.py b/gapro_amd/_lib.py
--- a/gapro_amd/_lib.py
+++ b/gapro_amd/_lib.py
@@ -104,6 +104,12 @@
                 ("point_count", C.c_void_p), ("feats_spp", C.c_void_p), ("occ_bits", C.c_void_p),
                 ("n_bbs", C.c_void_p), ("sem_spp", C.c_void_p), ("inst_spp", C.c_void_p), ("prob_spp", C.c_void_p),
                 ("sem", C.c_void_p), ("inst", C.c_void_p), ("prob", C.c_void_p)]
+
+
+class SceneLayout(C.Structure):
+    _fields_ = [("n_spps", C.c_int32), ("fixed_shift", C.c_int32), ("status", C.c_int32), ("reserved", C.c_int32),
+                ("feat_sum", C.c_int64), ("occ_count", C.c_int64), ("point_count", C.c_int64), ("feats_spp", C.c_int64),
+                ("occ_bits", C.c_int64), ("n_bbs", C.c_int64), ("feats_row_base", C.c_int64)]
 
 
 class PthArray(C.Structure):
@@ -302,6 +308,10 @@
     "gapro_partition_prepare_batch": (C.c_int, [_P, _P, C.c_int32, C.c_int32, _P, _P, _P, _P]),
     "gapro_partition_pool_batch": (C.c_int, [_P, _P, C.c_int32, C.c_int32, _P, _P]),
     "gapro_partition_pool_plan": (C.c_int, [C.c_int32, C.c_int32]),
+    "gapro_partition_layout": (C.c_int, [C.c_int32, C.c_int32, C.c_int32, _P, _P, _P, C.c_size_t, C.c_size_t, C.c_size_t,
+                                         _P, _P]),
+    "gapro_partition_pool_batch_dev": (C.c_int, [_P, _P, C.c_int32, C.c_int32, C.c_int32, _P, _P, _P, _P, _P, C.c_size_t,
+                                                 _P, C.c_size_t, _P, C.c_size_t, _P, _P]),
     "gapro_broadcast_labels_batch": (C.c_int, [_P, _P, C.c_int32, _P, _P]),
     "gapro_instance_info_workspace_bytes": (C.c_size_t, [C.c_int32]),
     "gapro_instance_info": (C.c_int, [_P, _P, C.c_int64, _P, _P, _P, C.c_int32, C.c_int32, _P, C.c_size_t, _P, _P, _P, _P,
diff --git a/gapro_amd/csrc/partition.hip b/gapro_amd/csrc/partition.hip
--- a/gapro_amd/csrc/partition.hip
+++ b/gapro_amd/csrc/partition.hip
@@ -204,6 +204,106 @@
     spp_inv[i] = (int)rank[spp[i] - smin];
 }
 
+__host__ __device__ inline unsigned long long align16(unsigned long long x) { return (x + 15ull) & ~15ull; }
+
+__host__ __device__ inline void layout_sizes(long long S, int B, int d, int pc_in_tables, unsigned long long* tal,
+                                             unsigned long long* tab) {
+  const unsigned long long s = (unsigned long long)S, W = (unsigned long long)((B + 63) / 64);
+  *tal = align16(s * (8ull * d + 4ull * B + (pc_in_tables ? 0ull : 4ull)));
+  *tab = align16(s * (8ull * W + 4ull + (pc_in_tables ? 4ull : 0ull)));
+}
+
+__host__ __device__ inline gapro_scene_layout layout_record(long long S, int B, int d, int pc_in_tables,
+                                                            unsigned long long tal_off, unsigned long long tab_off,
+                                                            unsigned long long row_base, int fixed_shift, int status) {
+  const unsigned long long s = (unsigned long long)S, W = (unsigned long long)((B + 63) / 64);
+  gapro_scene_layout r;
+  r.n_spps = (int32_t)S; r.fixed_shift = fixed_shift; r.status = status; r.reserved = 0;
+  r.feat_sum = (int64_t)tal_off;
+  r.occ_count = (int64_t)(tal_off + 8ull * s * d);
+  r.occ_bits = (int64_t)tab_off;
+  r.n_bbs = (int64_t)(tab_off + 8ull * s * W);
+  r.point_count = pc_in_tables ? (int64_t)(tab_off + 8ull * s * W + 4ull * s)
+                               : (int64_t)(tal_off + 8ull * s * d + 4ull * s * B);
+  r.feats_spp = (int64_t)(4ull * d * row_base);
+  r.feats_row_base = (int64_t)row_base;
+  return r;
+}
+
+__device__ inline unsigned long long block_exclusive_scan64(unsigned long long v, unsigned long long* total) {
+  __shared__ unsigned long long wsum64[kThreads / 64];
+  const int lane = threadIdx.x & 63, w = threadIdx.x >> 6;
+  unsigned long long inc = v;
+  for (int o = 1; o < 64; o <<= 1) {
+    const unsigned long long t = __shfl_up(inc, o, 64);
+    if (lane >= o) inc += t;
+  }
+  if (lane == 63) wsum64[w] = inc;
+  __syncthreads();
+  unsigned long long base = 0, tot = 0;
+  for (int j = 0; j < kThreads / 64; ++j) {
+    if (j < w) base += wsum64[j];
+    tot += wsum64[j];
+  }
+  __syncthreads();
+  *total = tot;
+  return base + inc - v;
+}
+
+struct PoolArenas {
+  char* tallies; char* tables; char* feats;
+  unsigned long long cap_tallies, cap_tables, cap_feats;
+};
+
+__global__ __launch_bounds__(kThreads) void k_pool_layout(gapro_scene_task* __restrict__ tasks,
+                                                          const gapro_scene_header* __restrict__ headers,
+                                                          const double* __restrict__ ground_h, int n_scenes, int d,
+                                                          int pc_in_tables, PoolArenas a,
+                                                          gapro_scene_layout* __restrict__ layouts) {
+  unsigned long long tal_tot = 0, tab_tot = 0, row_tot = 0;
+  for (int c0 = 0; c0 < n_scenes; c0 += kThreads) {
+    const int i = c0 + threadIdx.x;
+    long long S = 0;
+    int B = 1, shift = 0, status = GAPRO_OK;
+    if (i < n_scenes) {
+      const gapro_scene_header& h = headers[i];
+      status = h.status; shift = h.fixed_shift;
+      B = tasks[i].n_boxes;
+      S = status == GAPRO_OK ? (long long)h.n_spps : 0ll;
+    }
+    unsigned long long tal, tab, t0, t1, t2;
+    layout_sizes(S, B, d, pc_in_tables, &tal, &tab);
+    const unsigned long long tal_off = tal_tot + block_exclusive_scan64(tal, &t0);
+    const unsigned long long tab_off = tab_tot + block_exclusive_scan64(tab, &t1);
+    const unsigned long long row_base = row_tot + block_exclusive_scan64((unsigned long long)S, &t2);
+    tal_tot += t0; tab_tot += t1; row_tot += t2;
+    if (i < n_scenes) layouts[i] = layout_record(S, B, d, pc_in_tables, tal_off, tab_off, row_base, shift, status);
+  }
+  const bool overflow = tal_tot > a.cap_tallies || tab_tot > a.cap_tables || row_tot * 4ull * d > a.cap_feats;
+  for (int i = threadIdx.x; i < n_scenes; i += kThreads) {
+    gapro_scene_layout r = layouts[i];
+    gapro_scene_task& t = tasks[i];
+    if (overflow) {
+      r.n_spps = 0; r.status = GAPRO_ERR_WORKSPACE;
+      layouts[i] = r;
+    }
+    t.n_spps = r.n_spps;
+    t.fixed_shift = r.fixed_shift;
+    t.feat_sum = (int64_t*)(a.tallies + r.feat_sum);
+    t.occ_count = (int32_t*)(a.tallies + r.occ_count);
+    t.point_count = (int32_t*)((pc_in_tables ? a.tables : a.tallies) + r.point_count);
+    t.feats_spp = (float*)(a.feats + r.feats_spp);
+    t.occ_bits = (uint64_t*)(a.tables + r.occ_bits);
+    t.n_bbs = (int32_t*)(a.tables + r.n_bbs);
+    if (r.n_spps > 0) {
+      const gapro_scene_header& h = headers[i];
+      double* row = (double*)t.boxes + 6 * (size_t)(t.n_boxes - 1);
+      row[0] = h.coord_min[0]; row[1] = h.coord_min[1]; row[2] = h.coord_min[2];
+      row[3] = h.coord_max[0]; row[4] = h.coord_max[1]; row[5] = h.coord_min[2] + ground_h[i];
+    }
+  }
+}
+
 __global__ __launch_bounds__(kThreads) void k_pool_clear(const gapro_scene_task* __restrict__ tasks, int d) {
   const gapro_scene_task& t = tasks[blockIdx.y];
   const long long S = t.n_spps, nf = S * d, no = S * t.n_boxes;
@@ -217,6 +317,7 @@
 
 __global__ __launch_bounds__(kThreads) void k_pool(const gapro_scene_task* __restrict__ tasks, int d) {
   const gapro_scene_task& t = tasks[blockIdx.y];
+  if (t.n_spps <= 0) return;
   const long long n = t.n_points;
   const int nb = t.n_boxes, shift = t.fixed_shift;
   const double* __restrict__ coords = t.coords;
@@ -254,7 +355,7 @@
   const gapro_scene_task& t = tasks[blockIdx.y];
   const long long n = t.n_points;
   const long long p0 = (long long)blockIdx.x * kPoolRun;
-  if (p0 >= n) return;
+  if (p0 >= n || t.n_spps <= 0) return;
   const long long p1 = p0 + kPoolRun < n ? p0 + kPoolRun : n;
   const int nb = t.n_boxes, shift = t.fixed_shift;
   const double* __restrict__ coords = t.coords;
@@ -362,26 +463,26 @@
   float* __restrict__ feats_spp = t.feats_spp;
   unsigned long long* __restrict__ occ_bits = (unsigned long long*)t.occ_bits;
   int* __restrict__ n_bbs = t.n_bbs;
-  const int s = blockIdx.x * kThreads + threadIdx.x;
-  if (s >= n_spps) return;
-  const int pc = point_count[s] > 0 ? point_count[s] : 1;
-  const float pcf = (float)pc;
-  const int words = (nb + 63) / 64;
-  int nbb = 0;
-  for (int w = 0; w < words; ++w) {
-    unsigned long long bits = 0;
-    const int b_end = min(nb, (w + 1) * 64);
-    for (int b = w * 64; b < b_end; ++b) {
-      const float mean = (float)occ_count[(long long)s * nb + b] / pcf;
-      if (mean >= thresh) bits |= 1ull << (b - w * 64);
+  for (int s = blockIdx.x * kThreads + threadIdx.x; s < n_spps; s += gridDim.x * kThreads) {
+    const int pc = point_count[s] > 0 ? point_count[s] : 1;
+    const float pcf = (float)pc;
+    const int words = (nb + 63) / 64;
+    int nbb = 0;
+    for (int w = 0; w < words; ++w) {
+      unsigned long long bits = 0;
+      const int b_end = min(nb, (w + 1) * 64);
+      for (int b = w * 64; b < b_end; ++b) {
+        const float mean = (float)occ_count[(long long)s * nb + b] / pcf;
+        if (mean >= thresh) bits |= 1ull << (b - w * 64);
+      }
+      occ_bits[(long long)s * words + w] = bits;
+      nbb += __popcll(bits);
     }
-    occ_bits[(long long)s * words + w] = bits;
-    nbb += __popcll(bits);
-  }
-  n_bbs[s] = nbb;
-  const double pcd = (double)pc;
-  for (int k = 0; k < d; ++k)
-    feats_spp[(long long)s * d + k] = (float)fixed_mean(feat_sum[(long long)s * d + k], shift, pcd);
+    n_bbs[s] = nbb;
+    const double pcd = (double)pc;
+    for (int k = 0; k < d; ++k)
+      feats_spp[(long long)s * d + k] = (float)fixed_mean(feat_sum[(long long)s * d + k], shift, pcd);
+  }
 }
 
 __global__ __launch_bounds__(kThreads) void k_broadcast(const gapro_scene_task* __restrict__ tasks) {
@@ -476,6 +577,34 @@
   return lds + pool_table_bytes(feat_dim, n_boxes_max, log2_slots) <= 60 * 1024 ? log2_slots : 0;
 }
 
+static int launch_pool_kernels(gapro_ctx* ctx, hipStream_t stream, int32_t n_scenes, int32_t feat_dim,
+                               gapro_scene_task* d_tasks, long long n_max, int nb_max, long long clear_max,
+                               int fin_blocks) {
+  const int plan = gapro_partition_pool_plan(feat_dim, nb_max);
+  if (plan < 0) return gapro_fail(ctx, GAPRO_ERR_BAD_ARG, "gapro_partition_pool: too many boxes (%d)", nb_max);
+  const size_t lds = pool_box_bytes(nb_max);
+  const unsigned ny = (unsigned)n_scenes;
+  hipLaunchKernelGGL(k_pool_clear, dim3(grid_for(clear_max, 1, 256), ny), dim3(kThreads), 0, stream, d_tasks, (int)feat_dim);
+  if (plan > 0) {
+    const int log2_slots = plan;
+    const size_t lds2 = lds + pool_table_bytes(feat_dim, nb_max, log2_slots);
+    if (lds2 > 48 * 1024)
+      GAPRO_HIP_CHECK(ctx, hipFuncSetAttribute((const void*)k_pool_lds, hipFuncAttributeMaxDynamicSharedMemorySize,
+                                               (int)lds2));
+    const unsigned gx = (unsigned)((n_max + kPoolRun - 1) / kPoolRun);
+    hipLaunchKernelGGL(k_pool_lds, dim3(gx, ny), dim3(kThreads), lds2, stream, d_tasks, (int)feat_dim, log2_slots,
+                       nb_max);
+  } else {
+    const int cap = n_scenes >= 8 ? 512 : 4096;
+    hipLaunchKernelGGL(k_pool, dim3(grid_for(n_max * kLanesPerPoint, 1, cap), ny), dim3(kThreads), lds, stream, d_tasks,
+                       (int)feat_dim);
+  }
+  hipLaunchKernelGGL(k_pool_finalize, dim3((unsigned)fin_blocks, ny), dim3(kThreads), 0, stream, d_tasks,
+                     (int)feat_dim);
+  GAPRO_LAUNCH_CHECK(ctx);
+  return GAPRO_OK;
+}
+
 int gapro_partition_pool_batch(gapro_ctx* ctx, void* stream_, int32_t n_scenes, int32_t feat_dim,
                                const gapro_scene_task* h_tasks, gapro_scene_task* d_tasks) {
   int rc = check_tasks(ctx, "gapro_partition_pool_batch", n_scenes, h_tasks, d_tasks);
@@ -492,32 +621,68 @@
     s_max = std::max(s_max, (int)t.n_spps);
     clear_max = std::max<long long>(clear_max, (long long)t.n_spps * (feat_dim + t.n_boxes + 1));
   }
-  const int plan = gapro_partition_pool_plan(feat_dim, nb_max);
-  if (plan < 0) return gapro_fail(ctx, GAPRO_ERR_BAD_ARG, "gapro_partition_pool: too many boxes (%d)", nb_max);
-  const size_t lds = pool_box_bytes(nb_max);
   hipStream_t stream = (hipStream_t)stream_;
   GAPRO_HIP_CHECK(ctx, hipMemcpyAsync(d_tasks, h_tasks, (size_t)n_scenes * sizeof(gapro_scene_task),
                                       hipMemcpyHostToDevice, stream));
-  const unsigned ny = (unsigned)n_scenes;
-  hipLaunchKernelGGL(k_pool_clear, dim3(grid_for(clear_max, 1, 256), ny), dim3(kThreads), 0, stream, d_tasks, (int)feat_dim);
-  if (plan > 0) {
-    const int log2_slots = plan;
-    const size_t lds2 = lds + pool_table_bytes(feat_dim, nb_max, log2_slots);
-    if (lds2 > 48 * 1024)
-      GAPRO_HIP_CHECK(ctx, hipFuncSetAttribute((const void*)k_pool_lds, hipFuncAttributeMaxDynamicSharedMemorySize,
-                                               (int)lds2));
-    const unsigned gx = (unsigned)((n_max + kPoolRun - 1) / kPoolRun);
-    hipLaunchKernelGGL(k_pool_lds, dim3(gx, ny), dim3(kThreads), lds2, stream, d_tasks, (int)feat_dim, log2_slots,
-                       nb_max);
-  } else {
-    const int cap = n_scenes >= 8 ? 512 : 4096;
-    hipLaunchKernelGGL(k_pool, dim3(grid_for(n_max * kLanesPerPoint, 1, cap), ny), dim3(kThreads), lds, stream, d_tasks,
-                       (int)feat_dim);
-  }
-  hipLaunchKernelGGL(k_pool_finalize, dim3((s_max + kThreads - 1) / kThreads, ny), dim3(kThreads), 0, stream, d_tasks,
-                     (int)feat_dim);
+  return launch_pool_kernels(ctx, stream, n_scenes, feat_dim, d_tasks, n_max, nb_max, clear_max,
+                             (s_max + kThreads - 1) / kThreads);
+}
+
+int gapro_partition_layout(int32_t n_scenes, int32_t feat_dim, int32_t point_count_in_tables, const int32_t* h_n_spps,
+                           const int32_t* h_n_boxes, const int32_t* h_status, size_t cap_tallies, size_t cap_tables,
+                           size_t cap_feats, gapro_scene_layout* out, size_t* out_totals) {
+  if (n_scenes <= 0 || feat_dim <= 0 || !h_n_spps || !h_n_boxes || !h_status || !out) return GAPRO_ERR_BAD_ARG;
+  for (int i = 0; i < n_scenes; ++i)
+    if (h_n_boxes[i] <= 0 || (h_status[i] == GAPRO_OK && h_n_spps[i] < 0)) return GAPRO_ERR_BAD_ARG;
+  const int pl = point_count_in_tables ? 1 : 0;
+  unsigned long long tal_tot = 0, tab_tot = 0, row_tot = 0;
+  for (int i = 0; i < n_scenes; ++i) {
+    const long long S = h_status[i] == GAPRO_OK ? (long long)h_n_spps[i] : 0ll;
+    unsigned long long tal, tab;
+    layout_sizes(S, h_n_boxes[i], feat_dim, pl, &tal, &tab);
+    out[i] = layout_record(S, h_n_boxes[i], feat_dim, pl, tal_tot, tab_tot, row_tot, 0, h_status[i]);
+    tal_tot += tal; tab_tot += tab; row_tot += (unsigned long long)S;
+  }
+  if (out_totals) {
+    out_totals[0] = (size_t)tal_tot; out_totals[1] = (size_t)tab_tot; out_totals[2] = (size_t)(row_tot * 4ull * feat_dim);
+  }
+  if (tal_tot > cap_tallies || tab_tot > cap_tables || row_tot * 4ull * feat_dim > cap_feats) {
+    for (int i = 0; i < n_scenes; ++i) { out[i].n_spps = 0; out[i].status = GAPRO_ERR_WORKSPACE; }
+    return GAPRO_ERR_WORKSPACE;
+  }
+  return GAPRO_OK;
+}
+
+int gapro_partition_pool_batch_dev(gapro_ctx* ctx, void* stream_, int32_t n_scenes, int32_t feat_dim,
+                                   int32_t point_count_in_tables, const gapro_scene_task* h_tasks,
+                                   gapro_scene_task* d_tasks, const gapro_scene_header* d_headers,
+                                   const double* d_ground_h, void* d_tallies, size_t cap_tallies, void* d_tables,
+                                   size_t cap_tables, void* d_feats, size_t cap_feats, gapro_scene_layout* d_layouts,
+                                   gapro_scene_layout* h_layouts_pinned) {
+  int rc = check_tasks(ctx, "gapro_partition_pool_batch_dev", n_scenes, h_tasks, d_tasks);
+  if (rc != GAPRO_OK) return rc;
+  if (feat_dim <= 0 || !d_headers || !d_ground_h || !d_tallies || !d_tables || !d_feats || !d_layouts ||
+      !h_layouts_pinned)
+    return gapro_fail(ctx, GAPRO_ERR_BAD_ARG, "gapro_partition_pool_batch_dev: bad argument");
+  long long n_max = 0, clear_max = 0;
+  int nb_max = 0;
+  for (int i = 0; i < n_scenes; ++i) {
+    const gapro_scene_task& t = h_tasks[i];
+    if (t.n_points <= 0 || t.n_boxes <= 0 || !t.coords || !t.feats || !t.spp_inv || !t.boxes)
+      return gapro_fail(ctx, GAPRO_ERR_BAD_ARG, "gapro_partition_pool_batch_dev: scene %d: bad argument", i);
+    n_max = std::max<long long>(n_max, t.n_points);
+    nb_max = std::max(nb_max, (int)t.n_boxes);
+    clear_max = std::max<long long>(clear_max, t.n_points * (feat_dim + t.n_boxes + 1));
+  }
+  hipStream_t stream = (hipStream_t)stream_;
+  const PoolArenas a = {(char*)d_tallies, (char*)d_tables, (char*)d_feats, cap_tallies, cap_tables, cap_feats};
+  hipLaunchKernelGGL(k_pool_layout, dim3(1), dim3(kThreads), 0, stream, d_tasks, d_headers, d_ground_h, (int)n_scenes,
+                     (int)feat_dim, point_count_in_tables ? 1 : 0, a, d_layouts);
   GAPRO_LAUNCH_CHECK(ctx);
-  return GAPRO_OK;
+  GAPRO_HIP_CHECK(ctx, hipMemcpyAsync(h_layouts_pinned, d_layouts, (size_t)n_scenes * sizeof(gapro_scene_layout),
+                                      hipMemcpyDeviceToHost, stream));
+  return launch_pool_kernels(ctx, stream, n_scenes, feat_dim, d_tasks, n_max, nb_max, clear_max,
+                             grid_for(n_max, 1, 16));
 }
 
 int gapro_broadcast_labels_batch(gapro_ctx* ctx, void* stream_, int32_t n_scenes, const gapro_scene_task* h_tasks,
diff --git a/gapro_amd/fit_runner.py b/gapro_amd/fit_runner.py
--- a/gapro_amd/fit_runner.py
+++ b/gapro_amd/fit_runner.py
@@ -570,7 +570,7 @@
     def fit_launch(self, feats_spp, descs, n_fits: int, h_idx: np.ndarray, n_out: int,
                    init_mean: Optional[np.ndarray] = None, keep_debug: bool = False, slot: str = "s0",
                    scene_keys: Optional[Sequence[int]] = None, keep_models: bool = False,
-                   state_to_host: bool = True) -> PendingFit:
+                   state_to_host: bool = True, after=None) -> PendingFit:
         lib, ctx, be = self.lib, self.ctx, self.be
         D = int(feats_spp.shape[1])
         ws_bytes = int(lib.gapro_fit_plan_workspace(C.cast(descs, C.c_void_p), n_fits, D))
@@ -598,6 +598,8 @@
         prev = self._last_fit_done if self.serialize_fits else None
         if prev is not None:
             be.current_stream().wait_event(prev)
+        if after is not None:
+            be.current_stream().wait_event(after)
         args = (ctx.handle, self._sh(), n_fits, D, _ptr(feats_spp), _ptr(d_idx), C.cast(descs, C.c_void_p),
                 _ptr(d_descs), _ptr(d_init), C.byref(self.opt), _ptr(ws), ws_bytes, _ptr(o["probs"]),
                 _ptr(o["probs_new"]), _ptr(o["labels"]), _ptr(o["mu"]), _ptr(o["var"]), _ptr(s["status"]),
diff --git a/gapro_amd/pipeline.py b/gapro_amd/pipeline.py
--- a/gapro_amd/pipeline.py
+++ b/gapro_amd/pipeline.py
@@ -163,6 +163,10 @@
         self.stage_times = {}
         self._pin_events = {}
         self._keep = {}
+        self.fuse_partition = True
+        self._spp_density = None
+        self._pool_caps = (0, 0, 0)
+        self.pool_overflows = 0
 
 
     def _task_array(self, jobs: Sequence[SceneJob]):
@@ -193,6 +197,20 @@
             ev["end"] = self.be.event(enable_timing=True)
             ev["end"].record(self.be.current_stream())
             self.part_events.append(ev)
+
+    @staticmethod
+    def _static_boxes(job: SceneJob):
+        st = job.host.get("_static")
+        if st is None:
+            nw = len(job.wall_box)
+            st = (np.concatenate([job.instance_box.astype(np.float64), job.wall_box.astype(np.float64),
+                                  np.zeros((1, 6))], 0),
+                  np.ascontiguousarray(np.concatenate([job.instance_cls,
+                                                       np.full(nw + 1, job.instance_classes, dtype=np.int64)])),
+                  np.concatenate([job.instance_box_volume.astype(np.float64), job.wall_box_volume.astype(np.float64),
+                                  np.zeros(1)]))
+            dict.__setitem__(job.host, "_static", st)
+        return st
 
     def _prepare_finish(self, job: SceneJob, hdr: SceneHeader):
         if hdr.status != 0:
@@ -206,16 +224,7 @@
         job.header = hdr
         job.n_spps = int(hdr.n_spps)
         job.dev.pop("prep_ws", None)
-        st = job.host.get("_static")
-        if st is None:
-            nw = len(job.wall_box)
-            st = (np.concatenate([job.instance_box.astype(np.float64), job.wall_box.astype(np.float64),
-                                  np.zeros((1, 6))], 0),
-                  np.ascontiguousarray(np.concatenate([job.instance_cls,
-                                                       np.full(nw + 1, job.instance_classes, dtype=np.int64)])),
-                  np.concatenate([job.instance_box_volume.astype(np.float64), job.wall_box_volume.astype(np.float64),
-                                  np.zeros(1)]))
-            dict.__setitem__(job.host, "_static", st)
+        st = self._static_boxes(job)
         mn, mx = hdr.coord_min, hdr.coord_max
         boxes, vol = st[0].copy(), st[2].copy()
         boxes[-1] = (mn[0], mn[1], mn[2], mx[0], mx[1], mn[2] + job.ground_h)
@@ -227,8 +236,13 @@
         self._prepare_all([job])
 
     def _prepare_all(self, jobs: Sequence[SceneJob]):
+        tasks, d_tasks = self._task_array(jobs)
+        pinned, d_headers, prep_ws = self._prepare_enqueue(jobs, tasks, d_tasks)
+        self.be.current_stream().synchronize()
+        return self._prepare_collect(jobs, tasks, d_tasks, pinned)
+
+    def _prepare_enqueue(self, jobs: Sequence[SceneJob], tasks, d_tasks):
         lib, be = self.lib, self.be
-        tasks, d_tasks = self._task_array(jobs)
         D = int(jobs[0].feats.shape[1])
         caps = [int(self.spp_range_cap) if self.spp_range_cap else max(4 * j.n_points, 1 << 20) for j in jobs]
         ws_off, ws_tot = self._carve([lib.gapro_partition_prepare_workspace_bytes(j.n_points, c)
@@ -248,7 +262,11 @@
             self.ctx.handle, self._sh(), len(jobs), D, C.cast(tasks, C.c_void_p), _ptr(d_tasks),
             _ptr(d_headers), _ptr(pinned)))
         self._part_event_end(ev)
-        be.current_stream().synchronize()
+        return pinned, d_headers, prep_ws
+
+    def _prepare_collect(self, jobs: Sequence[SceneJob], tasks, d_tasks, pinned):
+        be = self.be
+        hsz = C.sizeof(SceneHeader)
         raw = pinned.numpy()
         for i, job in enumerate(jobs):
             self._prepare_finish(job, SceneHeader.from_buffer_copy(raw[i * hsz:(i + 1) * hsz].tobytes()))
@@ -388,14 +406,18 @@
         nxt = on(1, next, it, None)
         prev_state = None
         while cur_state is not None:
-            nxt_state = on(i + 1, self._partition, nxt, False) if nxt is not None else None
+            pend = on(i + 1, self._partition_enqueue, nxt, False) if nxt is not None else None
+            nxt_state = on(i + 1, self._partition, nxt, False) if nxt is not None and pend is None else None
             early = None
             if self.point_level and prev_state is not None:
                 early = on(i - 1, self._finish, prev_state, False)
             if i > 0:
-                on(i, self._launch, cur_state)
+                on(i, self._launch, cur_state, pend["done"] if pend is not None else None)
             if prev_state is not None:
                 yield early if early is not None else on(i - 1, self._finish, prev_state, False)
+            if pend is not None:
+                nxt_state = on(i + 1, self._partition_collect, pend)
+                pend = None
             nxt = on(i + 2, next, it, None) if nxt is not None else None
             if nxt_state is not None:
                 on(i + 1, self._schedule_all, nxt_state)
@@ -432,8 +454,11 @@
         _mark("start")
         all_jobs = list(jobs)
         tasks, d_tasks = self._prepare_all(jobs)
+        _mark("A prepare")
+        return self._partition_pool(all_jobs, tasks, d_tasks, stream, slot, _mark, keep_debug)
+
+    def _partition_pool(self, all_jobs, tasks, d_tasks, stream, slot, _mark, keep_debug):
         jobs = [j for j in all_jobs if j.error is None]
-        _mark("A prepare")
         if not jobs:
             return BatchState([], all_jobs, stream, slot, _mark, tasks, d_tasks, keep_debug)
         D = int(jobs[0].feats.shape[1])
@@ -443,6 +468,7 @@
                 raise ValueError("all scenes of a batch must share the feature dimension")
             job.feats_row_base = base
             base += job.n_spps
+        self._note_density(jobs)
         feats_spp_all = self.be.empty_typed((base, D), self.be.f32)
         need = sum(job.n_spps * (((job.n_boxes + 63) // 64) * 8 + 4 + (4 if self.point_level else 0)) + 16
                    for job in jobs)
@@ -451,6 +477,122 @@
         stream.synchronize()
         _mark("B pool")
         return BatchState(jobs, all_jobs, stream, slot, _mark, tasks, d_tasks, keep_debug, feats_spp_all=feats_spp_all)
+
+    kPoolHeadroom = 1.5
+
+    def _note_density(self, jobs):
+        r = sum(j.n_spps for j in jobs) / float(sum(j.n_points for j in jobs))
+        self._spp_density = max(self._spp_density or 0.0, r)
+
+    def _pool_capacity(self, jobs, D):
+        if not self._spp_density:
+            return None
+        n, pts = len(jobs), sum(j.n_points for j in jobs)
+        rows = min(int(self.kPoolHeadroom * self._spp_density * pts) + n, pts)
+        nb = max(len(j.instance_box) + len(j.wall_box) + 1 for j in jobs)
+        pl = 4 if self.point_level else 0
+        need = (rows * (8 * D + 4 * nb + 4 - pl) + 16 * n, rows * (8 * ((nb + 63) // 64) + 4 + pl) + 16 * n,
+                rows * 4 * D)
+        self._pool_caps = tuple(max(a, b) for a, b in zip(self._pool_caps, need))
+        return self._pool_caps
+
+    def _partition_enqueue(self, jobs: Sequence[SceneJob], keep_debug: bool = False):
+        lib, be = self.lib, self.be
+        all_jobs = list(jobs)
+        D = int(all_jobs[0].feats.shape[1])
+        if any(int(j.feats.shape[1]) != D for j in all_jobs):
+            raise ValueError("all scenes of a batch must share the feature dimension")
+        caps = self._pool_capacity(all_jobs, D) if self.fuse_partition else None
+        if caps is None:
+            return None
+        _mark = self._marker(jobs)
+        stream = be.current_stream()
+        slot = "s%x" % int(stream.cuda_stream)
+        _mark("start")
+        n = len(all_jobs)
+        tasks, d_tasks = self._task_array(all_jobs)
+        statics = [self._static_boxes(j) for j in all_jobs]
+        box_off, box_tot = self._carve([st[0].nbytes for st in statics], 64)
+        h_boxes = self._pinned("boxes" + slot[1:], box_tot + 8 * n)
+        hb = h_boxes.numpy()
+        for st, bo in zip(statics, box_off):
+            hb[bo:bo + st[0].nbytes] = st[0].view(np.uint8).reshape(-1)
+        hb[box_tot:box_tot + 8 * n] = np.array([j.ground_h for j in all_jobs], dtype=np.float64).view(np.uint8)
+        d_boxes = be.empty(box_tot + 8 * n)
+        d_boxes.copy_(h_boxes[:box_tot + 8 * n], non_blocking=True)
+        for t, job, st, bo in zip(tasks, all_jobs, statics, box_off):
+            t.boxes, t.n_boxes = d_boxes.data_ptr() + bo, len(st[0])
+            t.thresh_spp_occu = float(job.thresh_spp_occu)
+        pinned, d_headers, prep_ws = self._prepare_enqueue(all_jobs, tasks, d_tasks)
+        if self.serialize_fits and self._last_fit_done is not None:
+            stream.wait_event(self._last_fit_done)
+        cap_tal, cap_tab, cap_feats = caps
+        d_tallies, d_tables, d_feats = be.empty(cap_tal), be.empty(cap_tab), be.empty(cap_feats)
+        lsz = C.sizeof(_lib.SceneLayout)
+        d_layouts = be.empty(n * lsz)
+        h_layouts = self._pinned(slot + "layouts", n * lsz)
+        stage = self._pinned(slot + "tables", cap_tab)
+        ev = self._part_event(all_jobs, "pool")
+        self.ctx.check(lib.gapro_partition_pool_batch_dev(
+            self.ctx.handle, self._sh(), n, D, 1 if self.point_level else 0, C.cast(tasks, C.c_void_p), _ptr(d_tasks),
+            _ptr(d_headers), C.c_void_p(d_boxes.data_ptr() + box_tot), _ptr(d_tallies), cap_tal, _ptr(d_tables),
+            cap_tab, _ptr(d_feats), cap_feats, _ptr(d_layouts), _ptr(h_layouts)))
+        self._part_event_end(ev)
+        stage[:cap_tab].copy_(d_tables, non_blocking=True)
+        done = stream.record_event()
+        _mark("A+B enqueued")
+        return dict(all_jobs=all_jobs, tasks=tasks, d_tasks=d_tasks, stream=stream, slot=slot, mark=_mark,
+                    keep_debug=keep_debug, D=D, done=done, pinned=pinned, h_layouts=h_layouts, stage=stage,
+                    d_boxes=d_boxes, box_off=box_off, d_tallies=d_tallies, d_tables=d_tables, d_feats=d_feats,
+                    keep=(d_headers, prep_ws, d_layouts))
+
+    def _partition_collect(self, pend):
+        be = self.be
+        all_jobs, tasks, d_tasks, _mark = pend["all_jobs"], pend["tasks"], pend["d_tasks"], pend["mark"]
+        stream, slot, D = pend["stream"], pend["slot"], pend["D"]
+        if not pend["done"].query():
+            pend["done"].synchronize()
+        tasks, d_tasks = self._prepare_collect(all_jobs, tasks, d_tasks, pend["pinned"])
+        _mark("A prepare")
+        lsz = C.sizeof(_lib.SceneLayout)
+        raw = pend["h_layouts"].numpy()[:len(all_jobs) * lsz].tobytes()
+        recs = (_lib.SceneLayout * len(all_jobs)).from_buffer_copy(raw)
+        if any(r.status == _lib.GAPRO_ERR_WORKSPACE for r in recs):
+            self.pool_overflows += 1
+            return self._partition_pool(all_jobs, tasks, d_tasks, stream, slot, _mark, pend["keep_debug"])
+        jobs = [j for j in all_jobs if j.error is None]
+        if not jobs:
+            return BatchState([], all_jobs, stream, slot, _mark, tasks, d_tasks, pend["keep_debug"])
+        self._note_density(jobs)
+        pl = self.point_level
+        d_boxes, d_tallies, d_tables, stage = pend["d_boxes"], pend["d_tallies"], pend["d_tables"], pend["stage"]
+        feats_u8 = pend["d_feats"]
+        base = 0
+        for job, r, bo in zip(all_jobs, recs, pend["box_off"]):
+            if job.error is not None:
+                continue
+            S, B = job.n_spps, job.n_boxes
+            if r.n_spps != S or r.feats_row_base != base:
+                raise RuntimeError("layout record of a scene disagrees with its header")
+            W = (B + 63) // 64
+            d, h = job.dev, job.host
+            job.feats_row_base = base
+            base += S
+            d.spec("boxes", d_boxes, bo, job.boxes.nbytes, be.f64, (B, 6))
+            d.spec("feat_sum", d_tallies, r.feat_sum, 8 * S * D, be.i64, (S, D))
+            d.spec("occ_count", d_tallies, r.occ_count, 4 * S * B, be.i32, (S, B))
+            d.spec("point_count", d_tables if pl else d_tallies, r.point_count, 4 * S, be.i32, (S,))
+            d.spec("occ_bits", d_tables, r.occ_bits, 8 * S * W, be.i64, (S, W))
+            d.spec("n_bbs", d_tables, r.n_bbs, 4 * S, be.i32, (S,))
+            d.spec("feats_spp", feats_u8, r.feats_spp, 4 * S * D, be.f32, (S, D))
+            h.spec("occ_bits_pin", stage, r.occ_bits, 8 * S * W, be.i64, (S, W))
+            h.spec("n_bbs_pin", stage, r.n_bbs, 4 * S, be.i32, (S,))
+            if pl:
+                h.spec("point_count_pin", stage, r.point_count, 4 * S, be.i32, (S,))
+        feats_spp_all = feats_u8[:4 * base * D].view(be.f32).view(base, D)
+        _mark("B pool")
+        return BatchState(jobs, all_jobs, stream, slot, _mark, tasks, d_tasks, pend["keep_debug"],
+                          feats_spp_all=feats_spp_all)
 
     def _schedule_all(self, state: BatchState):
         lib = self.lib
@@ -483,10 +625,10 @@
         _mark("C export")
         state.n_fits, state.n_out, state.descs, state.h_idx = n_fits, n_out, descs, h_idx
 
-    def _launch(self, state: BatchState):
+    def _launch(self, state: BatchState, after=None):
         if state.n_fits:
             state.pending = self.fit_launch(state.feats_spp_all, state.descs, state.n_fits, state.h_idx, state.n_out,
-                                            keep_debug=state.keep_debug, slot=state.slot,
+                                            keep_debug=state.keep_debug, slot=state.slot, after=after,
                                             scene_keys=[j.scene_key for j in state.jobs],
                                             keep_models=state.keep_models or self.point_level,
                                             state_to_host=state.keep_models)
diff --git a/include/gapro_hip.h b/include/gapro_hip.h
--- a/include/gapro_hip.h
+++ b/include/gapro_hip.h
@@ -97,6 +97,31 @@
                                   gapro_scene_header* d_headers, gapro_scene_header* h_headers_pinned);
 int gapro_partition_pool_batch(gapro_ctx* ctx, void* stream, int32_t n_scenes, int32_t feat_dim,
                                const gapro_scene_task* h_tasks, gapro_scene_task* d_tasks);
+typedef struct {
+  int32_t n_spps;
+  int32_t fixed_shift;
+  int32_t status;
+  int32_t reserved;
+  int64_t feat_sum;
+  int64_t occ_count;
+  int64_t point_count;
+  int64_t feats_spp;
+  int64_t occ_bits;
+  int64_t n_bbs;
+  int64_t feats_row_base;
+} gapro_scene_layout;
+
+int gapro_partition_layout(int32_t n_scenes, int32_t feat_dim, int32_t point_count_in_tables, const int32_t* h_n_spps,
+                           const int32_t* h_n_boxes, const int32_t* h_status, size_t cap_tallies, size_t cap_tables,
+                           size_t cap_feats, gapro_scene_layout* out, size_t* out_totals);
+
+int gapro_partition_pool_batch_dev(gapro_ctx* ctx, void* stream, int32_t n_scenes, int32_t feat_dim,
+                                   int32_t point_count_in_tables, const gapro_scene_task* h_tasks,
+                                   gapro_scene_task* d_tasks, const gapro_scene_header* d_headers,
+                                   const double* d_ground_h, void* d_tallies, size_t cap_tallies, void* d_tables,
+                                   size_t cap_tables, void* d_feats, size_t cap_feats, gapro_scene_layout* d_layouts,
+                                   gapro_scene_layout* h_layouts_pinned);
+
 int gapro_partition_pool_plan(int32_t feat_dim, int32_t n_boxes_max);
 int gapro_broadcast_labels_batch(gapro_ctx* ctx, void* stream, int32_t n_scenes,
                                  const gapro_scene_task* h_tasks, gapro_scene_task* d_tasks);
```

Result: slower. 372.1 (-2.2%).
